# gitouni/Spatial-Temporal-LiDAR-camera-Calibration

Measured on NVIDIA B200. Metric: extrinsic_cost_evals_per_s, higher is better.
Workload: dtype f64

## Files before the change

### spatial-temporal-lidar-camera-calibration_b200/csrc/knn.cuh

```cuda
#pragma once
#include <cfloat>
#include <cmath>

#include "common.cuh"
#include "geom.cuh"
#include "kernels.h"

namespace stl {

constexpr unsigned kFull = 0xffffffffu;

struct ScanView {
    const float *px, *py, *pz;
    const uint32_t *orig;
    const float4 *lo, *hi;
    const uint16_t *adj;
    const float *adj_cov;
    unsigned long long *stats;
    int n0, n1;
};

__device__ __forceinline__ ScanView make_view(const DevPack &pk, const DevKf &K) {
    ScanView v;
    v.px = pk.px + K.pt_off; v.py = pk.py + K.pt_off; v.pz = pk.pz + K.pt_off;
    v.orig = pk.orig + K.pt_off;
    v.lo = pk.node_lo + K.node_off; v.hi = pk.node_hi + K.node_off;
    v.adj = pk.adj ? pk.adj + K.node_off * 32 : nullptr;
    v.adj_cov = pk.adj ? pk.adj_cov + K.node_off : nullptr;
    v.stats = nullptr;
    v.n0 = K.n0; v.n1 = K.n1;
    return v;
}

struct QueryF { float xl, xh, yl, yh, zl, zh; };
__device__ __forceinline__ QueryF make_queryf(double x, double y, double z) {
    QueryF q;
    q.xl = __double2float_rd(x); q.xh = __double2float_ru(x);
    q.yl = __double2float_rd(y); q.yh = __double2float_ru(y);
    q.zl = __double2float_rd(z); q.zh = __double2float_ru(z);
    return q;
}
__device__ __forceinline__ float box_lbf(const QueryF &q, float4 lo, float4 hi) {
    const float dx = fmaxf(fmaxf(__fsub_rd(lo.x, q.xh), __fsub_rd(q.xl, hi.x)), 0.f);
    const float dy = fmaxf(fmaxf(__fsub_rd(lo.y, q.yh), __fsub_rd(q.yl, hi.y)), 0.f);
    const float dz = fmaxf(fmaxf(__fsub_rd(lo.z, q.zh), __fsub_rd(q.zl, hi.z)), 0.f);
    const float s = __fadd_rd(__fadd_rd(__fmul_rd(dx, dx), __fmul_rd(dy, dy)), __fmul_rd(dz, dz));
    return __fmul_rd(s, 0.99999976f);
}

struct Sink1 {
    double d = DBL_MAX;
    float df = 3.402823466e+38f;
    float g2 = HUGE_VALF;
    uint32_t oi = 0xffffffffu, pos = 0xffffffffu;
    __device__ __forceinline__ bool may_contain(float lb) const { return lb <= df; }
    __device__ __forceinline__ static float below(double dd) { return __fmul_rd(__double2float_rd(dd), 0.99999976f); }
    __device__ __forceinline__ void note_pruned(float lb, bool pruned) {
        const unsigned k = __reduce_min_sync(kFull, pruned ? __float_as_uint(lb) : 0x7f800000u);
        g2 = fminf(g2, __uint_as_float(k));
    }
    __device__ __forceinline__ void note_bound(float b) { g2 = fminf(g2, b); }
    __device__ __forceinline__ void seed(const ScanView &S, uint32_t p, double qx, double qy, double qz) {
        const double dd = dist3e(qx, qy, qz, (double)S.px[p], (double)S.py[p], (double)S.pz[p]);
        if (dd == dd) { d = dd; df = __double2float_ru(dd); oi = S.orig[p]; pos = p; }
    }
    __device__ __forceinline__ void visit(const ScanView &S, int leaf, double qx, double qy, double qz, int lane) {
        const int g = leaf * kLeaf + lane;
        const double dd = dist3e(qx, qy, qz, (double)S.px[g], (double)S.py[g], (double)S.pz[g]);
        const float lowf = dd == dd ? below(dd) : __int_as_float(0x7f800000);
        const bool q = dd <= d;
        if (!__any_sync(kFull, q)) {
            note_pruned(lowf, (uint32_t)g != pos);
            return;
        }
        const uint32_t o = q ? S.orig[g] : 0xffffffffu;
        unsigned hi = q ? (unsigned)__double2hiint(dd) : 0xffffffffu;
        const unsigned mhi = __reduce_min_sync(kFull, hi);
        unsigned lo = (q && hi == mhi) ? (unsigned)__double2loint(dd) : 0xffffffffu;
        const unsigned mlo = __reduce_min_sync(kFull, lo);
        const bool tie = q && hi == mhi && (unsigned)__double2loint(dd) == mlo;
        const unsigned mo = __reduce_min_sync(kFull, tie ? o : 0xffffffffu);
        const double cd = __hiloint2double((int)mhi, (int)mlo);
        if (cd < d || (cd == d && mo < oi)) {
            const int src = __ffs(__ballot_sync(kFull, tie && o == mo)) - 1;
            if (pos != 0xffffffffu) g2 = fminf(g2, below(d));
            note_pruned(lowf, lane != src);
            d = cd; oi = mo; pos = (uint32_t)(leaf * kLeaf + src);
            df = __double2float_ru(cd);
        } else {
            note_pruned(lowf, (uint32_t)g != pos);
        }
    }
};

struct SinkK {
    double kd = DBL_MAX;
    uint32_t ki = 0xffffffffu, kpos = 0xffffffffu;
    int count = 0, k;
    double r2, wd;
    float r2f, wdf;
    uint32_t wi = 0xffffffffu;
    __device__ __forceinline__ SinkK(int k_, double r2_) : k(k_), r2(r2_), wd(r2_) {
        r2f = r2_ < 3.0e38 ? __double2float_ru(r2_) : 3.402823466e+38f;
        wdf = r2f;
    }
    __device__ __forceinline__ bool accept(double d, uint32_t i) const {
        return d < r2 && (count < k || d < wd || (d == wd && i < wi));
    }
    __device__ __forceinline__ bool may_contain(float lb) const { return lb <= r2f && (count < k || lb <= wdf); }
    __device__ __forceinline__ void note_pruned(float, bool) {}
    __device__ __forceinline__ void note_bound(float) {}
    __device__ __forceinline__ void visit(const ScanView &S, int leaf, double qx, double qy, double qz, int lane) {
        const int g = leaf * kLeaf + lane;
        const double dd = dist3e(qx, qy, qz, (double)S.px[g], (double)S.py[g], (double)S.pz[g]);
        const bool pre = dd < r2 && (count < k || dd <= wd);
        unsigned mask = __ballot_sync(kFull, pre);
        if (!mask) return;
        const uint32_t o = pre ? S.orig[g] : 0xffffffffu;
        if (__popc(mask) >= (count == 0 ? 4 : 8)) {
            bulk_merge(pre ? dd : (double)INFINITY, o, (uint32_t)g, lane);
            return;
        }
        while (mask) {
            const int src = __ffs(mask) - 1;
            mask &= mask - 1;
            const double cd = __shfl_sync(kFull, dd, src);
            const uint32_t ci = __shfl_sync(kFull, o, src);
            if (!accept(cd, ci)) continue;
            const bool less = lane < count && (kd < cd || (kd == cd && ki < ci));
            const int at = __popc(__ballot_sync(kFull, less));
            const double sd = __shfl_up_sync(kFull, kd, 1);
            const uint32_t si = __shfl_up_sync(kFull, ki, 1), sp = __shfl_up_sync(kFull, kpos, 1);
            if (lane > at) { kd = sd; ki = si; kpos = sp; }
            else if (lane == at) { kd = cd; ki = ci; kpos = (uint32_t)(leaf * kLeaf + src); }
            if (count < k) ++count;
            if (count == k) { wd = __shfl_sync(kFull, kd, k - 1); wi = __shfl_sync(kFull, ki, k - 1); wdf = __double2float_ru(wd); }
        }
    }

    __device__ __forceinline__ static void cx(double &d, uint32_t &i, uint32_t &p, int j, bool keep_min) {
        const double od = __shfl_xor_sync(kFull, d, j);
        const uint32_t oi = __shfl_xor_sync(kFull, i, j), op = __shfl_xor_sync(kFull, p, j);
        const bool other_less = od < d || (od == d && oi < i);
        const bool other_more = od > d || (od == d && oi > i);
        if (keep_min ? other_less : other_more) { d = od; i = oi; p = op; }
    }

    __device__ __forceinline__ void bulk_merge(double cd, uint32_t ci, uint32_t cp, int lane) {
        unsigned key = cd < (double)INFINITY ? ((__float_as_uint(__double2float_rd(cd)) & ~31u) | (unsigned)lane) : (0xffffffe0u | (unsigned)lane);
#pragma unroll
        for (int kk = 2; kk <= 32; kk <<= 1) {
#pragma unroll
            for (int j = kk >> 1; j > 0; j >>= 1) {
                const unsigned o = __shfl_xor_sync(kFull, key, j);
                const bool keep_min = ((lane & kk) == 0) == ((lane & j) == 0);
                key = keep_min ? min(key, o) : max(key, o);
            }
        }
        {
            const int src = (int)(key & 31u);
            const double sd = __shfl_sync(kFull, cd, src);
            const uint32_t si = __shfl_sync(kFull, ci, src), sp = __shfl_sync(kFull, cp, src);
            cd = sd; ci = si; cp = sp;
        }
        const unsigned next_key = __shfl_down_sync(kFull, key, 1);
        if (__ballot_sync(kFull, lane < 31 && (key >> 5) == (next_key >> 5) && cd < (double)INFINITY)) {
            for (;;) {
                bool moved = false;
#pragma unroll 1
                for (int parity = 0; parity < 2; ++parity) {
                    const bool lower = (lane & 1) == parity;
                    const int partner = lower ? lane + 1 : lane - 1;
                    const bool ok = partner >= 0 && partner < 32;
                    const double od = __shfl_sync(kFull, cd, ok ? partner : lane);
                    const uint32_t oi = __shfl_sync(kFull, ci, ok ? partner : lane), op = __shfl_sync(kFull, cp, ok ? partner : lane);
                    const bool other_less = od < cd || (od == cd && oi < ci);
                    const bool other_more = od > cd || (od == cd && oi > ci);
                    if (ok && (lower ? other_less : other_more)) { cd = od; ci = oi; cp = op; moved = true; }
                }
                if (!__any_sync(kFull, moved)) break;
            }
        }
        if (count == 0) {
            kd = cd; ki = ci; kpos = cp;
        } else {
            if (lane >= count) { kd = (double)INFINITY; ki = 0xffffffffu; }
            const double rd = __shfl_sync(kFull, cd, 31 - lane);
            const uint32_t ri = __shfl_sync(kFull, ci, 31 - lane), rp = __shfl_sync(kFull, cp, 31 - lane);
            if (rd < kd || (rd == kd && ri < ki)) { kd = rd; ki = ri; kpos = rp; }
#pragma unroll
            for (int j = 16; j > 0; j >>= 1) cx(kd, ki, kpos, j, (lane & j) == 0);
        }
        const int nvalid = __popc(__ballot_sync(kFull, kd < (double)INFINITY));
        count = nvalid < k ? nvalid : k;
        if (count == k) { wd = __shfl_sync(kFull, kd, k - 1); wi = __shfl_sync(kFull, ki, k - 1); wdf = __double2float_ru(wd); }
    }
};

template <class Sink>
__device__ __forceinline__ void traverse(const ScanView &S, double qx, double qy, double qz, Sink &sink, int lane, int first_leaf = -1) {
    if (first_leaf >= 0) sink.visit(S, first_leaf, qx, qy, qz, lane);
    const float4 *lo2 = S.lo + S.n0 + S.n1, *hi2 = S.hi + S.n0 + S.n1;
    const float4 *lo1 = S.lo + S.n0, *hi1 = S.hi + S.n0;
    const QueryF qf = make_queryf(qx, qy, qz);
    const float lb2 = box_lbf(qf, lo2[lane], hi2[lane]);
    const unsigned key2 = __float_as_uint(lb2);
    unsigned done2 = 0;
    for (;;) {
        const bool c2 = !((done2 >> lane) & 1u) && sink.may_contain(lb2);
        const unsigned m2 = __reduce_min_sync(kFull, c2 ? key2 : 0xffffffffu);
        if (m2 == 0xffffffffu) break;
        const int s2 = __ffs(__ballot_sync(kFull, c2 && key2 == m2)) - 1;
        done2 |= 1u << s2;
        const int n1i = s2 * 32 + lane;
        const float lb1 = box_lbf(qf, lo1[n1i], hi1[n1i]);
        const unsigned key1 = __float_as_uint(lb1);
        unsigned done1 = 0;
        for (;;) {
                const bool c1 = !((done1 >> lane) & 1u) && sink.may_contain(lb1);
            const unsigned m1 = __reduce_min_sync(kFull, c1 ? key1 : 0xffffffffu);
            if (m1 == 0xffffffffu) break;
            const int s1 = __ffs(__ballot_sync(kFull, c1 && key1 == m1)) - 1;
            done1 |= 1u << s1;
            const int n0i = (s2 * 32 + s1) * 32 + lane;
            const float lb0 = box_lbf(qf, S.lo[n0i], S.hi[n0i]);
            const unsigned key0 = __float_as_uint(lb0);
            unsigned done0 = ((s2 * 32 + s1) == (first_leaf >> 5) && first_leaf >= 0) ? (1u << (first_leaf & 31)) : 0u;
            for (;;) {
                        const bool c0 = !((done0 >> lane) & 1u) && sink.may_contain(lb0);
                const unsigned m0 = __reduce_min_sync(kFull, c0 ? key0 : 0xffffffffu);
                if (m0 == 0xffffffffu) break;
                const int s0 = __ffs(__ballot_sync(kFull, c0 && key0 == m0)) - 1;
                done0 |= 1u << s0;
                sink.visit(S, (s2 * 32 + s1) * 32 + s0, qx, qy, qz, lane);
            }
            sink.note_pruned(lb0, !((done0 >> lane) & 1u));
        }
        sink.note_pruned(lb1, !((done1 >> lane) & 1u));
    }
    sink.note_pruned(lb2, !((done2 >> lane) & 1u));
}

__device__ __forceinline__ int next_ticket(int *ticket, int lane) {
    int t = 0;
    if (lane == 0) t = atomicAdd(ticket, 1);
    return __shfl_sync(kFull, t, 0);
}

template <class Sink>
__device__ __forceinline__ float scan_adjacent(const ScanView &S, int home, double qx, double qy, double qz, Sink &sink, int lane) {
    if (S.adj == nullptr) return -1.f;
    const float cov = S.adj_cov[home];
    if (cov < 0.f) return -1.f;
    const unsigned id = S.adj[(long long)home * 32 + lane];
    const QueryF qf = make_queryf(qx, qy, qz);
    const float lb = id != 0xffffu ? box_lbf(qf, S.lo[id], S.hi[id]) : __int_as_float(0x7f800000);
    const unsigned key = __float_as_uint(lb);
    unsigned done = 0;
    for (;;) {
        const bool c = !((done >> lane) & 1u) && sink.may_contain(lb);
        const unsigned m = __reduce_min_sync(kFull, c ? key : 0xffffffffu);
        if (m == 0xffffffffu) break;
        const int s = __ffs(__ballot_sync(kFull, c && key == m)) - 1;
        done |= 1u << s;
        sink.visit(S, (int)__shfl_sync(kFull, id, s), qx, qy, qz, lane);
    }
    sink.note_pruned(lb, !((done >> lane) & 1u));
    return cov;
}

__device__ __forceinline__ void knn_around_point(const ScanView &S, uint32_t pos, SinkK &kn, int lane) {
    const double x = (double)S.px[pos], y = (double)S.py[pos], z = (double)S.pz[pos];
    const float cov = scan_adjacent(S, (int)(pos >> 5), x, y, z, kn, lane);
    const bool done = cov > 3.0e38f || (cov >= 0.f && kn.count == kn.k && kn.wdf < cov);
    if (S.stats && lane == 0) { atomicAdd(S.stats + 0, 1ull); atomicAdd(S.stats + (done ? 1 : (cov >= 0.f ? 2 : 3)), 1ull); }
    if (done) return;
    if (cov >= 0.f) kn = SinkK(kn.k, kn.r2);
    traverse(S, x, y, z, kn, lane, (int)(pos >> 5));
}

__device__ __forceinline__ float home_box_delta(const ScanView &S, int home, double qx, double qy, double qz) {
    const float4 lo = S.lo[home], hi = S.hi[home];
    const float xl = __double2float_rd(qx), xh = __double2float_ru(qx), yl = __double2float_rd(qy), yh = __double2float_ru(qy);
    const float zl = __double2float_rd(qz), zh = __double2float_ru(qz);
    const float gx = fmaxf(fmaxf(__fsub_ru(lo.x, xl), __fsub_ru(xh, hi.x)), 0.f);
    const float gy = fmaxf(fmaxf(__fsub_ru(lo.y, yl), __fsub_ru(yh, hi.y)), 0.f);
    const float gz = fmaxf(fmaxf(__fsub_ru(lo.z, zl), __fsub_ru(zh, hi.z)), 0.f);
    return __fsqrt_ru(__fadd_ru(__fadd_ru(__fmul_ru(gx, gx), __fmul_ru(gy, gy)), __fmul_ru(gz, gz)));
}

__device__ __forceinline__ void nn_near_leaf_seeded(const ScanView &S, float adj_r, int home, double qx, double qy, double qz, Sink1 &nn,
                                                    int lane, float delta) {
    const float cov = scan_adjacent(S, home, qx, qy, qz, nn, lane);
    if (S.stats && lane == 0) atomicAdd(S.stats + 4, 1ull);
    if (cov >= 0.f && nn.pos != 0xffffffffu) {
        const float reach = __fadd_ru(__fsqrt_ru(nn.df), delta);
        if (cov > 3.0e38f ? reach <= adj_r : reach < __fsqrt_rd(cov)) {
            if (S.stats && lane == 0) atomicAdd(S.stats + 5, 1ull);
            const float u = __fsub_rd(cov > 3.0e38f ? adj_r : __fsqrt_rd(cov), delta);
            nn.note_bound(u > 0.f ? __fmul_rd(u, u) : 0.f);
            return;
        }
        const int l1 = (int)(nn.pos >> 5);
        if (l1 != home) {
            const float cov1 = S.adj_cov[l1];
            const float two_rho = __fmul_ru(2.f, __fsqrt_ru(nn.df));
            if (cov1 >= 0.f && (cov1 > 3.0e38f ? two_rho <= adj_r : two_rho < __fsqrt_rd(cov1))) {
                const float rho_up = __fsqrt_ru(nn.df);
                scan_adjacent(S, l1, qx, qy, qz, nn, lane);
                if (S.stats && lane == 0) atomicAdd(S.stats + 5, 1ull);
                const float u = __fsub_rd(cov1 > 3.0e38f ? adj_r : __fsqrt_rd(cov1), rho_up);
                nn.note_bound(u > 0.f ? __fmul_rd(u, u) : 0.f);
                return;
            }
        }
    }
    if (S.stats && lane == 0) atomicAdd(S.stats + (cov >= 0.f ? 6 : 7), 1ull);
    traverse(S, qx, qy, qz, nn, lane);
}

__device__ __forceinline__ void nn_near_leaf(const ScanView &S, float adj_r, int home, double qx, double qy, double qz, Sink1 &nn,
                                             int lane, uint32_t hint = 0xffffffffu) {
    if (hint != 0xffffffffu) nn.seed(S, hint, qx, qy, qz);
    nn_near_leaf_seeded(S, adj_r, home, qx, qy, qz, nn, lane, home_box_delta(S, home, qx, qy, qz));
}

struct PlaneOut { V3 n; double reg; int m; bool gates_ok; };

struct NbGather {
    const ScanView &S;
    const uint32_t *__restrict__ nb;
    __device__ __forceinline__ void get(int j, double &x, double &y, double &z) const {
        const uint32_t p = nb[j];
        x = (double)S.px[p]; y = (double)S.py[p]; z = (double)S.pz[p];
    }
};
struct NbCoords {
    const float4 *__restrict__ base;
    long long stride;
    __device__ __forceinline__ void get(int j, double &x, double &y, double &z) const {
        const float4 v = base[(long long)j * stride];
        x = (double)v.x; y = (double)v.y; z = (double)v.z;
    }
};
__device__ __forceinline__ void store_nb_coords(float4 *__restrict__ nbx, long long stride, long long slot, const ScanView &S, int lane,
                                                int count, uint32_t kpos) {
    float4 v = make_float4(0.f, 0.f, 0.f, 0.f);
    if (lane < count) v = make_float4(S.px[kpos], S.py[kpos], S.pz[kpos], __uint_as_float(kpos));
    nbx[(long long)lane * stride + slot] = v;
}

template <class Src>
__device__ __forceinline__ PlaneOut plane_fit(const Src &src, int m, double last, double cx, double cy, double cz, const DevParams &pr,
                                              const bool stable = false) {
    PlaneOut out;
    out.m = m;
    out.n = {0.0, 0.0, 0.0};
    out.reg = 0;
    out.gates_ok = false;
    if (stable) {
        if (m < 3) return out;
    } else if (m == 0 || (last < pr.min_diff2) || (m < pr.min_pts)) {
        return out;
    }
    out.gates_ok = true;
    double c0 = 0, c1 = 0, c2 = 0, c3 = 0, c4 = 0, c5 = 0, c6 = 0, c7 = 0, c8 = 0;
    for (int j = 0; j < m; ++j) {
        double x, y, z;
        src.get(j, x, y, z);
        c0 += x; c1 += y; c2 += z;
        c3 += x * x; c4 += x * y; c5 += x * z;
        c6 += y * y; c7 += y * z; c8 += z * z;
    }
    const double dm = (double)m;
    c0 /= dm; c1 /= dm; c2 /= dm; c3 /= dm; c4 /= dm; c5 /= dm; c6 /= dm; c7 /= dm; c8 /= dm;
    const double cov[6] = {c3 - c0 * c0, c4 - c0 * c1, c5 - c0 * c2, c6 - c1 * c1, c7 - c1 * c2, c8 - c2 * c2};
    const V3 n = normalized(smallest_eigvec(cov));
    double reg = 0;
    for (int j = 0; j < m; ++j) {
        double x, y, z;
        src.get(j, x, y, z);
        const V3 d = {x - cx, y - cy, z - cz};
        reg += fabs(dot(d, n));
    }
    out.n = n;
    out.reg = reg / (double)(m - 1);
    if (stable && sqrt(last) < pr.min_diff) out.reg = __longlong_as_double(0x7ff0000000000000ll);
    return out;
}


__device__ __forceinline__ PlaneOut plane_thread(const ScanView &S, const uint32_t *__restrict__ nb, int m, double last, double cx,
                                                 double cy, double cz, const DevParams &pr, const bool stable = false) {
    return plane_fit(NbGather{S, nb}, m, last, cx, cy, cz, pr, stable);
}

__device__ __forceinline__ PlaneOut plane_lookup(const DevPack &pk, const DevKf &K, uint32_t pos) {
    const PlaneRec r = pk.pl_rec[K.pt_off + pos];
    const int mm = pk.pl_m[K.pt_off + pos];
    PlaneOut out;
    out.gates_ok = mm >= 0;
    out.m = mm >= 0 ? mm : -(mm + 1);
    out.n = {r.nx, r.ny, r.nz};
    out.reg = r.reg;
    return out;
}

}
```

### spatial-temporal-lidar-camera-calibration_b200/csrc/knn3d.cu

```cuda
#include <algorithm>
#include <cstdlib>

#include "kernels.h"
#include "knn.cuh"

namespace stl {
namespace {

constexpr int kWarps = 8;
#ifndef STL_KNN_MINB
#define STL_KNN_MINB 8
#endif
constexpr int kPlaneThreads = 128;
#ifndef STL_PLANE_MINB
#define STL_PLANE_MINB 5
#endif

__device__ __forceinline__ void map_point_lidar(const DevPack &pk, const DevKf &K, const DevCand &c, int f, uint32_t kp, double &qx,
                                                double &qy, double &qz) {
    const float *Tcw = pk.Tcw + (long long)f * 12;
    const float *mp = pk.kp_mp + (K.kp_off + kp) * 3;
    const double wx = (double)__fmul_rn(mp[0], c.sf), wy = (double)__fmul_rn(mp[1], c.sf), wz = (double)__fmul_rn(mp[2], c.sf);
    const double cxm = dadd(dot3e((double)Tcw[0], (double)Tcw[1], (double)Tcw[2], wx, wy, wz), dmul((double)Tcw[3], c.s));
    const double cym = dadd(dot3e((double)Tcw[4], (double)Tcw[5], (double)Tcw[6], wx, wy, wz), dmul((double)Tcw[7], c.s));
    const double czm = dadd(dot3e((double)Tcw[8], (double)Tcw[9], (double)Tcw[10], wx, wy, wz), dmul((double)Tcw[11], c.s));
    xform(c.Ri, c.ti, cxm, cym, czm, qx, qy, qz);
}

__global__ void __launch_bounds__(kWarps * 32, STL_KNN_MINB)
k_nn_knn(const DevPack pk, const DevWork wk, const DevParams pr, const int B, const int batch, uint32_t *__restrict__ lm_pos,
         int *__restrict__ lm_m) {
    const int sub = wk.sub;
    const int j = blockIdx.x % sub;
    const int bf = blockIdx.x / sub;
    const int fi = bf / B, f = sel_kf(pk, fi), b = bf - fi * B;
    const int nq = wk.n_q[(long long)b * pk.n_kf + f];
    if (nq <= 0) return;
    const int lane = threadIdx.x & 31;
    const DevKf K = pk.kf[f];
    const DevCand &c = wk.cand[b];
    ScanView S = make_view(pk, K);
    S.stats = wk.dbg_stats;
    const long long cbase = (long long)b * pk.n_kp_total + K.kp_off;
    const long long qbase = (long long)b * pk.n_mp_total + K.mp_off;
    __shared__ int ticket;
    if (threadIdx.x == 0) ticket = 0;
    __syncthreads();
    for (;;) {
        const int t0 = next_ticket(&ticket, lane) * batch;
        if ((long long)t0 * sub + j >= nq) break;
        const int qi = (t0 + lane) * sub + j;
        const bool valid = lane < batch && qi < nq;
        double qx = 0, qy = 0, qz = 0, sd = DBL_MAX;
        uint32_t hint = 0, soi = 0xffffffffu, spos = 0xffffffffu;
        float delta = 0.f;
        if (valid) {
            const uint2 ks = wk.q_kpsp[cbase + qi];
            hint = ks.y;
            map_point_lidar(pk, K, c, f, ks.x, qx, qy, qz);
            const double dd = dist3e(qx, qy, qz, (double)S.px[hint], (double)S.py[hint], (double)S.pz[hint]);
            if (dd == dd) { sd = dd; soi = S.orig[hint]; spos = hint; }
            delta = home_box_delta(S, (int)(hint >> 5), qx, qy, qz);
        }
        uint32_t out_pos = 0xffffffffu;
        float out_g2 = 0.f;
        unsigned todo = __ballot_sync(kFull, valid);
        while (todo) {
            const int src = __ffs(todo) - 1;
            todo &= todo - 1;
            const double x = __shfl_sync(kFull, qx, src), y = __shfl_sync(kFull, qy, src), z = __shfl_sync(kFull, qz, src);
            const uint32_t h = __shfl_sync(kFull, hint, src);
            Sink1 nn;
            nn.d = __shfl_sync(kFull, sd, src);
            nn.oi = __shfl_sync(kFull, soi, src);
            nn.pos = __shfl_sync(kFull, spos, src);
            if (nn.pos != 0xffffffffu) nn.df = __double2float_ru(nn.d);
            nn_near_leaf_seeded(S, pr.adj_r, (int)(h >> 5), x, y, z, nn, lane, __shfl_sync(kFull, delta, src));
            if (lane == src) { out_pos = nn.pos; out_g2 = nn.g2; }
            if (pr.use_plane && !pr.plane_index) {
                const long long slot = qbase + (long long)(t0 + src) * sub + j;
                SinkK kn(pr.k, pr.radius2);
                knn_around_point(S, nn.pos, kn, lane);
                wk.nb[slot * kMaxK + lane] = lane < kn.count ? kn.kpos : 0xffffffffu;
                store_nb_coords(wk.nbx, wk.nbx_stride, slot, S, lane, kn.count, kn.kpos);
                const double last = __shfl_sync(kFull, kn.kd, kn.count > 0 ? kn.count - 1 : 0);
                if (lane == 0) { wk.nb_m[slot] = kn.count; wk.nb_last[slot] = last; }
            }
        }
        if (valid) { wk.nn_pos[qbase + qi] = out_pos; wk.nn_g2[qbase + qi] = out_g2; }
        if (lm_pos != nullptr && b == 0) {
            double lx = 0, ly = 0, lz = 0, nn_d = DBL_MAX;
            uint32_t nn_p = 0xffffffffu;
            bool need = false;
            if (valid) {
                const float *Tcw = pk.Tcw + (long long)f * 12;
                const float *mp = pk.kp_mp + (K.kp_off + wk.q_kpsp[cbase + qi].x) * 3;
                const double ma = (double)mp[0], mb = (double)mp[1], mc = (double)mp[2];
                const double Mx = dadd(dot3e((double)Tcw[0], (double)Tcw[1], (double)Tcw[2], ma, mb, mc), (double)Tcw[3]);
                const double My = dadd(dot3e((double)Tcw[4], (double)Tcw[5], (double)Tcw[6], ma, mb, mc), (double)Tcw[7]);
                const double Mz = dadd(dot3e((double)Tcw[8], (double)Tcw[9], (double)Tcw[10], ma, mb, mc), (double)Tcw[11]);
                xform(c.Ri, c.ti, dmul(Mx, c.s), dmul(My, c.s), dmul(Mz, c.s), lx, ly, lz);
                need = true;
                if (out_pos != 0xffffffffu) {
                    const double move = sqrt(dist3e(qx, qy, qz, lx, ly, lz)) * (1.0 + 1e-9) + 1e-12;
                    const double dh = dist3e(lx, ly, lz, (double)S.px[out_pos], (double)S.py[out_pos], (double)S.pz[out_pos]);
                    const double reach = (double)__fsqrt_rd(out_g2) - move;
                    if (reach > 0.0 && reach * reach > dh * (1.0 + 1e-6) + 1e-18) { need = false; nn_p = out_pos; nn_d = dh; }
                }
            }
            unsigned todo2 = __ballot_sync(kFull, need);
            while (todo2) {
                const int src = __ffs(todo2) - 1;
                todo2 &= todo2 - 1;
                const double x = __shfl_sync(kFull, lx, src), y = __shfl_sync(kFull, ly, src), z = __shfl_sync(kFull, lz, src);
                uint32_t h = __shfl_sync(kFull, out_pos, src);
                if (h == 0xffffffffu) h = __shfl_sync(kFull, hint, src);
                Sink1 nn;
                nn_near_leaf(S, pr.adj_r, (int)(h >> 5), x, y, z, nn, lane, h);
                if (lane == src) { nn_p = nn.pos; nn_d = nn.d; }
            }
            if (valid) {
                const long long slot = K.mp_off + qi;
                if (nn_d > pr.max_3d_dist2) {
                    lm_pos[slot] = 0xffffffffu;
                } else {
                    lm_pos[slot] = nn_p;
                    lm_m[slot] = nn_p == hint ? -2 : -3;
                }
            }
        }
    }
}

__global__ void __launch_bounds__(kPlaneThreads, STL_PLANE_MINB)
k_plane_dist(const DevPack pk, const DevWork wk, const DevParams pr, const int B, const int debug) {
    const int sub = wk.sub;
    const int j = blockIdx.x % sub;
    const int bf = blockIdx.x / sub;
    const int fi = bf / B, f = sel_kf(pk, fi), b = bf - fi * B;
    const long long rec = (long long)b * pk.n_kf + f;
    const int nq = wk.n_q[rec];
    double s3d = 0, v3d = 0, c3d = 0, vpl = 0, vpt = 0;
    if (nq > 0) {
        const DevKf K = pk.kf[f];
        const DevCand &c = wk.cand[b];
        const ScanView S = make_view(pk, K);
        const long long cbase = (long long)b * pk.n_kp_total + K.kp_off;
        const long long qbase = (long long)b * pk.n_mp_total + K.mp_off;
        for (int qi = j * kPlaneThreads + threadIdx.x; qi < nq; qi += sub * kPlaneThreads) {
            const uint32_t kp = wk.corr_kp[cbase + wk.q_corr[cbase + qi]];
            double qx, qy, qz;
            map_point_lidar(pk, K, c, f, kp, qx, qy, qz);
            const uint32_t np = wk.nn_pos[qbase + qi];
            const double nx = (double)S.px[np], ny = (double)S.py[np], nz = (double)S.pz[np];
            const double dx = dsub(nx, qx), dy = dsub(ny, qy), dz = dsub(nz, qz);
            double dist = sqrt(dot3e(dx, dy, dz, dx, dy, dz));
            int is_plane = 0, m = 0;
            if (pr.use_plane) {
                const PlaneOut po = pr.plane_index ? plane_lookup(pk, K, np)
                                                   : plane_fit(NbCoords{wk.nbx + qbase + qi, wk.nbx_stride}, wk.nb_m[qbase + qi], wk.nb_last[qbase + qi], nx, ny, nz, pr, pr.variant == 1);
                m = po.m;
                if (po.gates_ok && !(po.reg > pr.reg_thr)) {
                    is_plane = 1;
                    dist = fabs(dot3e(dx, dy, dz, po.n.x, po.n.y, po.n.z));
                }
            }
            if (dist < pr.thr3d) {
                s3d += dist; v3d += 1.0;
                if (is_plane) vpl += 1.0; else vpt += 1.0;
            }
            c3d += 1.0;
            if (debug) {
                const long long o = K.kp_off + qi;
                wk.dbg_nn[o] = S.orig[np];
                wk.dbg_m[o] = m;
                wk.dbg_plane[o] = is_plane;
                wk.dbg_dist[o] = dist;
                for (int t = 0; t < kMaxK; ++t) {
                    const uint32_t p = (pr.use_plane && !pr.plane_index && t < m) ? wk.nb[(qbase + qi) * kMaxK + t] : 0xffffffffu;
                    wk.dbg_knn[o * kMaxK + t] = p == 0xffffffffu ? 0xffffffffu : S.orig[p];
                }
            }
        }
    }
    __shared__ double red[5][kPlaneThreads / 32];
    const int lane = threadIdx.x & 31, warp = threadIdx.x >> 5;
    for (int o = 16; o; o >>= 1) {
        s3d += __shfl_down_sync(0xffffffffu, s3d, o); v3d += __shfl_down_sync(0xffffffffu, v3d, o);
        c3d += __shfl_down_sync(0xffffffffu, c3d, o); vpl += __shfl_down_sync(0xffffffffu, vpl, o);
        vpt += __shfl_down_sync(0xffffffffu, vpt, o);
    }
    if (lane == 0) { red[0][warp] = s3d; red[1][warp] = v3d; red[2][warp] = c3d; red[3][warp] = vpl; red[4][warp] = vpt; }
    __syncthreads();
    if (threadIdx.x == 0) {
        AlignRec r = {0, 0, 0, 0, 0};
        for (int w = 0; w < kPlaneThreads / 32; ++w) { r.s3d += red[0][w]; r.v3d += red[1][w]; r.c3d += red[2][w]; r.vpl += red[3][w]; r.vpt += red[4][w]; }
        wk.align[rec * sub + j] = r;
    }
}

__global__ void __launch_bounds__(kWarps * 32)
k_knn3d(const DevPack pk, const int kf, const double *__restrict__ q, const int nq, const int k, const double radius2,
        uint32_t *__restrict__ out_idx, double *__restrict__ out_d2, int *__restrict__ out_cnt) {
    const int lane = threadIdx.x & 31;
    const int qi = blockIdx.x * kWarps + (threadIdx.x >> 5);
    if (qi >= nq) return;
    const DevKf K = pk.kf[kf];
    const ScanView S = make_view(pk, K);
    SinkK kn(k, radius2 > 0 ? radius2 : DBL_MAX);
    traverse(S, q[qi * 3], q[qi * 3 + 1], q[qi * 3 + 2], kn, lane);
    if (lane < k) {
        out_idx[(long long)qi * k + lane] = lane < kn.count ? kn.ki : 0xffffffffu;
        out_d2[(long long)qi * k + lane] = lane < kn.count ? kn.kd : INFINITY;
    }
    if (lane == 0) out_cnt[qi] = kn.count;
}

__global__ void __launch_bounds__(kWarps * 32, STL_KNN_MINB)
k_index_knn(const DevPack pk, const int kf_begin, const DevParams pr, const long long first_pt, uint32_t *__restrict__ nb,
            int *__restrict__ nb_m, double *__restrict__ nb_last) {
    const DevKf K = pk.kf[kf_begin + blockIdx.y];
    const int lane = threadIdx.x & 31, warp = threadIdx.x >> 5;
    const ScanView S = make_view(pk, K);
    for (int p = blockIdx.x * kWarps + warp; p < K.n_pts; p += gridDim.x * kWarps) {
        SinkK kn(pr.k, pr.radius2);
        knn_around_point(S, (uint32_t)p, kn, lane);
        const long long o = K.pt_off - first_pt + p;
        nb[o * kMaxK + lane] = lane < kn.count ? kn.kpos : 0xffffffffu;
        const double last = __shfl_sync(kFull, kn.kd, kn.count > 0 ? kn.count - 1 : 0);
        if (lane == 0) { nb_m[o] = kn.count; nb_last[o] = last; }
    }
}

__global__ void __launch_bounds__(kPlaneThreads)
k_index_plane(const DevPack pk, const int kf_begin, const DevParams pr, const long long first_pt, const uint32_t *__restrict__ nb,
              const int *__restrict__ nb_m, const double *__restrict__ nb_last) {
    const DevKf K = pk.kf[kf_begin + blockIdx.y];
    const ScanView S = make_view(pk, K);
    for (int p = blockIdx.x * kPlaneThreads + threadIdx.x; p < K.n_pad; p += gridDim.x * kPlaneThreads) {
        PlaneRec r = {0.0, 0.0, 0.0, 0.0};
        int mm = -1;
        if (p < K.n_pts) {
            const long long o = K.pt_off - first_pt + p;
            const PlaneOut po = plane_thread(S, nb + o * kMaxK, nb_m[o], nb_last[o], (double)S.px[p], (double)S.py[p], (double)S.pz[p], pr, pr.variant == 1);
            r.nx = po.n.x; r.ny = po.n.y; r.nz = po.n.z; r.reg = po.reg;
            mm = po.gates_ok ? po.m : -(po.m + 1);
        }
        pk.pl_rec[K.pt_off + p] = r;
        pk.pl_m[K.pt_off + p] = mm;
    }
}

}

cudaError_t build_plane_index(const DevPack &pk, const DevKf *h_kf, int kf_begin, int nkf, const DevParams &pr, cudaStream_t st,
                              BuildScratch &scr) {
    const long long first = h_kf[kf_begin].pt_off;
    const long long npts = h_kf[kf_begin + nkf - 1].pt_off + h_kf[kf_begin + nkf - 1].n_pad - first;
    if (npts <= 0) return cudaSuccess;
    int max_pts = 0;
    for (int f = 0; f < nkf; ++f) max_pts = max_pts > h_kf[kf_begin + f].n_pad ? max_pts : h_kf[kf_begin + f].n_pad;
    cudaError_t e = scr.need(2, 4 * (size_t)npts * kMaxK);
    if (e == cudaSuccess) e = scr.need(4, 4 * (size_t)npts);
    if (e == cudaSuccess) e = scr.need(3, 8 * (size_t)npts);
    if (e != cudaSuccess) return e;
    uint32_t *nb = (uint32_t *)scr.buf[2]; int *m = (int *)scr.buf[4]; double *last = (double *)scr.buf[3];
    const int bx = (max_pts + kWarps * 16 - 1) / (kWarps * 16);
    k_index_knn<<<dim3(bx, nkf), kWarps * 32, 0, st>>>(pk, kf_begin, pr, first, nb, m, last);
    k_index_plane<<<dim3((max_pts + kPlaneThreads * 4 - 1) / (kPlaneThreads * 4), nkf), kPlaneThreads, 0, st>>>(pk, kf_begin, pr, first, nb, m, last);
    return cudaGetLastError();
}

namespace {
__global__ void k_debug_trig(const double *__restrict__ x, int n, double *__restrict__ ac, double *__restrict__ co) {
    const int i = blockIdx.x * blockDim.x + threadIdx.x;
    if (i >= n) return;
    ac[i] = acos_cr(fmin(fmax(x[i], -1.0), 1.0));
    co[i] = cos_cr(x[i]);
}
}

cudaError_t launch_debug_trig(const double *d_x, int n, double *d_acos, double *d_cos, cudaStream_t st) {
    if (n <= 0) return cudaSuccess;
    k_debug_trig<<<(n + 255) / 256, 256, 0, st>>>(d_x, n, d_acos, d_cos);
    return cudaGetLastError();
}

cudaError_t launch_align3d(const DevPack &pk, const DevWork &wk, const DevParams &pr, int B, int debug, cudaStream_t st, cudaEvent_t after_traversal,
                           uint32_t *lm_pos, int *lm_m) {
    if (B <= 0) return cudaSuccess;
    if (pk.n_sel <= 0) return after_traversal ? cudaEventRecord(after_traversal, st) : cudaSuccess;
    int batch = (long long)pk.n_sel * B >= 600 ? 8 : 4;
    if (const char *e = getenv("STL_K2_BATCH")) batch = std::max(1, std::min(32, atoi(e)));
    k_nn_knn<<<(unsigned)(pk.n_sel * B * wk.sub), kWarps * 32, 0, st>>>(pk, wk, pr, B, batch, lm_pos, lm_m);
    cudaError_t e = cudaGetLastError();
    if (e != cudaSuccess) return e;
    if (after_traversal && (e = cudaEventRecord(after_traversal, st)) != cudaSuccess) return e;
    k_plane_dist<<<(unsigned)(pk.n_sel * B * wk.sub), kPlaneThreads, 0, st>>>(pk, wk, pr, B, debug);
    return cudaGetLastError();
}

cudaError_t launch_knn3d(const DevPack &pk, int kf, const double *d_q, int nq, int k, double radius2, uint32_t *d_idx, double *d_d2,
                         int *d_cnt, cudaStream_t st) {
    if (nq <= 0) return cudaSuccess;
    k_knn3d<<<(nq + kWarps - 1) / kWarps, kWarps * 32, 0, st>>>(pk, kf, d_q, nq, k, radius2, d_idx, d_d2, d_cnt);
    return cudaGetLastError();
}

}
```

### spatial-temporal-lidar-camera-calibration_b200/csrc/lm.cu

```cuda
#include <cub/cub.cuh>

#include "../../include/stlcalib.h"
#include "dual.cuh"
#include "gprfit.hpp"
#include "knn.cuh"
#include "lm.h"

namespace stl {
namespace {

constexpr int kWarps = 8;
#ifndef STL_LM_MINB
#define STL_LM_MINB 6
#endif
constexpr int kLinVals = 41;
constexpr int kGprWarps = 1;
constexpr int kLinThreads = 128;


__device__ __forceinline__ void lm_lane(const DevPack &pk, DevWork &wk, LmState &lm, bool arg0 = true) {
    const int2 am = arg0 && blockIdx.y == 0 ? lm.lane0 : lm.amap[blockIdx.y];
    const long long nk = pk.n_kp_total, F = pk.n_kf, nm = lm.n_slots;
    const long long wc = am.x, wq = wc * nm;
    wk.cand += wc;
    wk.corr_kp += wc * nk; wk.corr_sp += wc * nk; wk.q_corr += wc * nk; wk.q_kpsp += wc * nk;
    wk.n_corr += wc * F; wk.n_q += wc * F;
    wk.nn_pos += wq; wk.nn_g2 += wq; wk.nb += wq * kMaxK; wk.nbx += wq; wk.nb_m += wq; wk.nb_last += wq;
    const long long lo = (long long)blockIdx.y * nm;
    lm.stage += lo; lm.plane_a += lo * 4; lm.nnb_pos += lo; lm.nbb += lo * kMaxK; lm.nbbx += lo; lm.nbb_m += lo; lm.nbb_last += lo;
    const long long po = (long long)am.y * lm.slot_stride;
    lm.slot_kf += po; lm.slot_kp += po; lm.flag2d += po; lm.type3d += po; lm.flag3d += po; lm.flagG += po;
    lm.geo2d += po * 6; lm.geo3d += po * 9; lm.gpr_nb += po * kMaxK; lm.gpr_m += po;
    lm.d_counts += am.y * 4;
}

__global__ void k_lm_clear(LmState lm) {
    const long long po = (long long)lm.amap[blockIdx.y].y * lm.slot_stride, n = lm.slot_stride, ptot = (long long)lm.P * n;
    for (long long i = (long long)blockIdx.x * blockDim.x + threadIdx.x; i < n; i += (long long)gridDim.x * blockDim.x) {
        lm.flags[po + i] = 0; lm.flags[ptot + po + i] = 0; lm.flags[2 * ptot + po + i] = 0; lm.flags[3 * ptot + po + i] = 0;
    }
    if (blockIdx.x == 0 && threadIdx.x < 4) lm.d_counts[lm.amap[blockIdx.y].y * 4 + threadIdx.x] = 0;
}

__device__ __forceinline__ bool lm_frame_active(const DevWork &wk, const DevParams &pr, int f, int &nq) {
    nq = wk.n_q[f];
    return wk.n_corr[f] >= pr.num_min_corr && nq > 0;
}

__device__ __forceinline__ void lm_map_point(const DevPack &pk, const DevKf &K, int f, uint32_t kp, double &Mx, double &My, double &Mz) {
    const float *Tcw = pk.Tcw + (long long)f * 12;
    const float *mp = pk.kp_mp + (K.kp_off + kp) * 3;
    const double a = (double)mp[0], b = (double)mp[1], c = (double)mp[2];
    Mx = dadd(dot3e((double)Tcw[0], (double)Tcw[1], (double)Tcw[2], a, b, c), (double)Tcw[3]);
    My = dadd(dot3e((double)Tcw[4], (double)Tcw[5], (double)Tcw[6], a, b, c), (double)Tcw[7]);
    Mz = dadd(dot3e((double)Tcw[8], (double)Tcw[9], (double)Tcw[10], a, b, c), (double)Tcw[11]);
}

__global__ void __launch_bounds__(kWarps * 32, STL_LM_MINB)
k_lm_knn_a(const DevPack pk, DevWork wk, const DevParams pr, LmState lm) {
    lm_lane(pk, wk, lm);
    const int j = blockIdx.x % lm.sub, f = sel_kf(pk, blockIdx.x / lm.sub);
    int nq;
    if (!lm_frame_active(wk, pr, f, nq)) return;
    const int lane = threadIdx.x & 31, warp = threadIdx.x >> 5;
    const DevKf K = pk.kf[f];
    const ScanView S = make_view(pk, K);
    const int C = pk.n_covis;
    __shared__ int ticket;
    if (threadIdx.x == 0) ticket = 0;
    __syncthreads();
    for (;;) {
        const int qi = next_ticket(&ticket, lane) * lm.sub + j;
        if (qi >= nq) break;
        const uint2 ks = wk.q_kpsp[K.kp_off + qi];
        const uint32_t kp = ks.x, sp = ks.y;
        const long long slot = K.mp_off + qi;
        const bool obs = lane < C && pk.covis_valid[f * C + lane] && !isnan(pk.covis_uv[(K.kp_off + kp) * C + lane].x);
        const int ncov = __popc(__ballot_sync(kFull, obs));
        if (ncov == 0) {
            if (lane == 0) wk.nb_m[slot] = -1;
            continue;
        }
        if (pr.plane_index && !pr.use_gpr) {
            if (lane == 0) wk.nb_m[slot] = 0;
            continue;
        }
        SinkK kn(pr.k, pr.radius2);
        knn_around_point(S, sp, kn, lane);
        wk.nb[slot * kMaxK + lane] = lane < kn.count ? kn.kpos : 0xffffffffu;
        store_nb_coords(wk.nbx, wk.nbx_stride, slot, S, lane, kn.count, kn.kpos);
        const double last = __shfl_sync(kFull, kn.kd, kn.count > 0 ? kn.count - 1 : 0);
        if (lane == 0) { wk.nb_m[slot] = kn.count; wk.nb_last[slot] = last; }
    }
}

__global__ void __launch_bounds__(128)
k_lm_plane_a(const DevPack pk, DevWork wk, const DevParams pr, LmState lm) {
    lm_lane(pk, wk, lm);
    const int j = blockIdx.x % lm.sub, f = sel_kf(pk, blockIdx.x / lm.sub);
    int nq;
    if (!lm_frame_active(wk, pr, f, nq)) return;
    __shared__ int cnt[2];
    if (threadIdx.x < 2) cnt[threadIdx.x] = 0;
    __syncthreads();
    const DevKf K = pk.kf[f];
    const ScanView S = make_view(pk, K);
    const bool from_index = pr.plane_index && !pr.use_gpr;
    const int C = pk.n_covis;
    for (int qi = j * blockDim.x + threadIdx.x; qi < nq; qi += lm.sub * blockDim.x) {
        const long long slot = K.mp_off + qi;
        lm.stage[slot] = 0;
        const uint32_t ci = wk.q_corr[K.kp_off + qi];
        const uint32_t kp = wk.corr_kp[K.kp_off + ci], sp = wk.corr_sp[K.kp_off + ci];
        int m = 0;
        if (from_index) {
            bool any = false;
            for (int s = 0; s < C; ++s) any = any || (pk.covis_valid[f * C + s] && !isnan(pk.covis_uv[(K.kp_off + kp) * C + s].x));
            if (!any) continue;
        } else {
            m = wk.nb_m[slot];
            if (m < 0) continue;
        }
        const double cx = (double)S.px[sp], cy = (double)S.py[sp], cz = (double)S.pz[sp];
        const PlaneOut po = from_index ? plane_lookup(pk, K, sp)
                                       : plane_fit(NbCoords{wk.nbx + slot, wk.nbx_stride}, m, wk.nb_last[slot], cx, cy, cz, pr);
        if (!po.gates_ok) continue;
        const long long cs = slot;
        lm.slot_kf[cs] = f;
        lm.slot_kp[cs] = kp;
        double *pa = lm.plane_a + slot * 4;
        pa[0] = po.n.x; pa[1] = po.n.y; pa[2] = po.n.z; pa[3] = po.reg;
        if (po.reg < pr.reg_thr) {
            double *g = lm.geo2d + cs * 6;
            g[0] = cx; g[1] = cy; g[2] = cz; g[3] = po.n.x; g[4] = po.n.y; g[5] = po.n.z;
            lm.flag2d[cs] = 1;
            atomicAdd(&cnt[0], 1);
        } else if (pr.use_gpr) {
            for (int t = 0; t < kMaxK; ++t) lm.gpr_nb[slot * kMaxK + t] = wk.nb[slot * kMaxK + t];
            lm.gpr_m[slot] = po.m;
            lm.flagG[cs] = 1;
            atomicAdd(&cnt[1], 1);
        }
        lm.stage[slot] = 1;
    }
    __syncthreads();
    if (threadIdx.x < 2 && cnt[threadIdx.x] > 0) atomicAdd(lm.d_counts + 3 * threadIdx.x, cnt[threadIdx.x]);
}

__global__ void __launch_bounds__(kWarps * 32, STL_LM_MINB)
k_lm_knn_b(const DevPack pk, DevWork wk, const DevParams pr, LmState lm, const bool hints, const bool cert) {
    lm_lane(pk, wk, lm);
    const uint32_t *__restrict__ nn_hint = hints ? wk.nn_pos : nullptr;
    const float *__restrict__ nn_g2 = hints && cert ? wk.nn_g2 : nullptr;
    const int j = blockIdx.x % lm.sub, f = sel_kf(pk, blockIdx.x / lm.sub);
    int nq;
    if (!lm_frame_active(wk, pr, f, nq)) return;
    const int lane = threadIdx.x & 31;
    const DevKf K = pk.kf[f];
    const DevCand &c0 = wk.cand[0];
    const ScanView S = make_view(pk, K);
    const float *Tcw = pk.Tcw + (long long)f * 12;
    __shared__ int ticket;
    if (threadIdx.x == 0) ticket = 0;
    __syncthreads();
    for (;;) {
        const int base = next_ticket(&ticket, lane) * 32;
        if ((long long)base * lm.sub + j >= nq) break;
        const int qi = (base + lane) * lm.sub + j;
        const long long slot = K.mp_off + qi;
        const bool valid = qi < nq && lm.stage[slot] == 1;
        uint32_t sp = 0, hint = 0xffffffffu, nn_pos = 0xffffffffu;
        double qx = 0, qy = 0, qz = 0, nn_d = DBL_MAX;
        bool settled = false;
        if (valid) {
            const uint2 ks = wk.q_kpsp[K.kp_off + qi];
            const uint32_t kp = ks.x;
            sp = ks.y;
            double Mx, My, Mz;
            lm_map_point(pk, K, f, kp, Mx, My, Mz);
            xform(c0.Ri, c0.ti, dmul(Mx, c0.s), dmul(My, c0.s), dmul(Mz, c0.s), qx, qy, qz);
            hint = nn_hint ? nn_hint[slot] : sp;
            if (hint == 0xffffffffu) hint = sp;
            if (nn_hint && nn_g2 && nn_hint[slot] != 0xffffffffu) {
                const float *mp = pk.kp_mp + (K.kp_off + kp) * 3;
                const double wx = (double)__fmul_rn(mp[0], c0.sf), wy = (double)__fmul_rn(mp[1], c0.sf), wz = (double)__fmul_rn(mp[2], c0.sf);
                const double ex = dadd(dot3e((double)Tcw[0], (double)Tcw[1], (double)Tcw[2], wx, wy, wz), dmul((double)Tcw[3], c0.s));
                const double ey = dadd(dot3e((double)Tcw[4], (double)Tcw[5], (double)Tcw[6], wx, wy, wz), dmul((double)Tcw[7], c0.s));
                const double ez = dadd(dot3e((double)Tcw[8], (double)Tcw[9], (double)Tcw[10], wx, wy, wz), dmul((double)Tcw[11], c0.s));
                double ox, oy, oz;
                xform(c0.Ri, c0.ti, ex, ey, ez, ox, oy, oz);
                const double move = sqrt(dist3e(ox, oy, oz, qx, qy, qz)) * (1.0 + 1e-9) + 1e-12;
                const double dh = dist3e(qx, qy, qz, (double)S.px[hint], (double)S.py[hint], (double)S.pz[hint]);
                const double reach = (double)__fsqrt_rd(nn_g2[slot]) - move;
                if (reach > 0.0 && reach * reach > dh * (1.0 + 1e-6) + 1e-18) { settled = true; nn_pos = hint; nn_d = dh; }
            }
        }
        unsigned todo = __ballot_sync(kFull, valid && !settled);
        while (todo) {
            const int src = __ffs(todo) - 1;
            todo &= todo - 1;
            const double sx = __shfl_sync(kFull, qx, src), sy = __shfl_sync(kFull, qy, src), sz = __shfl_sync(kFull, qz, src);
            const uint32_t sh = __shfl_sync(kFull, hint, src);
            Sink1 nn;
            nn_near_leaf(S, pr.adj_r, (int)(sh >> 5), sx, sy, sz, nn, lane, sh);
            if (lane == src) { nn_pos = nn.pos; nn_d = nn.d; }
        }
        bool want_knn = false;
        if (valid) {
            if (nn_d > pr.max_3d_dist2) {
                lm.nnb_pos[slot] = 0xffffffffu;
            } else {
                lm.nnb_pos[slot] = nn_pos;
                if (nn_pos == sp) lm.nbb_m[slot] = -2;
                else if (pr.plane_index) lm.nbb_m[slot] = -3;
                else want_knn = true;
            }
        }
        unsigned kn_todo = __ballot_sync(kFull, want_knn);
        while (kn_todo) {
            const int src = __ffs(kn_todo) - 1;
            kn_todo &= kn_todo - 1;
            const uint32_t p = __shfl_sync(kFull, nn_pos, src);
            const long long sl = K.mp_off + ((long long)(base + src) * lm.sub + j);
            SinkK kn(pr.k, pr.radius2);
            knn_around_point(S, p, kn, lane);
            lm.nbb[sl * kMaxK + lane] = lane < kn.count ? kn.kpos : 0xffffffffu;
            store_nb_coords(lm.nbbx, lm.nbbx_stride, sl, S, lane, kn.count, kn.kpos);
            const double last = __shfl_sync(kFull, kn.kd, kn.count > 0 ? kn.count - 1 : 0);
            if (lane == 0) { lm.nbb_m[sl] = kn.count; lm.nbb_last[sl] = last; }
        }
    }
}

__device__ __forceinline__ bool block3d_geometry(const DevPack &pk, const DevParams &pr, const LmState &lm, long long slot, int f, uint32_t kp,
                                                 double g[9], int &type) {
    if (lm.stage[slot] != 1) return false;
    const uint32_t np = lm.nnb_pos[slot];
    if (np == 0xffffffffu) return false;
    const DevKf &K = pk.kf[f];
    const float *sx = pk.px + K.pt_off, *sy = pk.py + K.pt_off, *sz = pk.pz + K.pt_off;
    const double nx = (double)sx[np], ny = (double)sy[np], nz = (double)sz[np];
    bool gates_ok, state;
    double n3[3];
    const int m = lm.nbb_m[slot];
    if (m == -2) {
        const double *pa = lm.plane_a + slot * 4;
        gates_ok = true; n3[0] = pa[0]; n3[1] = pa[1]; n3[2] = pa[2];
        state = pa[3] < pr.reg_thr;
    } else {
        const PlaneOut p2 = m == -3 ? plane_lookup(pk, K, np) : plane_fit(NbCoords{lm.nbbx + slot, lm.nbbx_stride}, m, lm.nbb_last[slot], nx, ny, nz, pr);
        gates_ok = p2.gates_ok; n3[0] = p2.n.x; n3[1] = p2.n.y; n3[2] = p2.n.z;
        state = p2.gates_ok && p2.reg < pr.reg_thr;
    }
    lm_map_point(pk, K, f, kp, g[0], g[1], g[2]);
    g[3] = nx; g[4] = ny; g[5] = nz;
    g[6] = gates_ok ? n3[0] : 0.0; g[7] = gates_ok ? n3[1] : 0.0; g[8] = gates_ok ? n3[2] : 1.0;
    type = state ? 2 : 1;
    return true;
}

__global__ void __launch_bounds__(128)
k_lm_plane_b(const DevPack pk, DevWork wk, const DevParams pr, LmState lm) {
    lm_lane(pk, wk, lm, false);
    const int j = blockIdx.x % lm.sub, f = sel_kf(pk, blockIdx.x / lm.sub);
    int nq;
    if (!lm_frame_active(wk, pr, f, nq)) return;
    const DevKf K = pk.kf[f];
    __shared__ int cnt[2];
    if (threadIdx.x < 2) cnt[threadIdx.x] = 0;
    __syncthreads();
    for (int qi = j * blockDim.x + threadIdx.x; qi < nq; qi += lm.sub * blockDim.x) {
        const long long slot = K.mp_off + qi;
        if (lm.stage[slot] != 1) continue;
        if (lm.nnb_pos[slot] == 0xffffffffu) continue;
        const uint32_t ci = wk.q_corr[K.kp_off + qi];
        const uint32_t kp = wk.corr_kp[K.kp_off + ci];
        double g9[9];
        int type;
        if (!block3d_geometry(pk, pr, lm, slot, f, kp, g9, type)) continue;
        double *g = lm.geo3d + slot * 9;
#pragma unroll
        for (int i = 0; i < 9; ++i) g[i] = g9[i];
        lm.type3d[slot] = (uint8_t)type;
        lm.flag3d[slot] = 1;
        atomicAdd(&cnt[0], 1);
        if (type == 1) atomicAdd(&cnt[1], 1);
    }
    __syncthreads();
    if (threadIdx.x < 2 && cnt[threadIdx.x] > 0) atomicAdd(lm.d_counts + 1 + threadIdx.x, cnt[threadIdx.x]);
}

struct Acc {
    double v[kLinVals];
};

struct F7 {
    double a;
    double v[7];
};
static_assert(sizeof(F7) == sizeof(D7), "F7 views D7 storage");
__device__ __forceinline__ F7 f7_const(double x) { F7 r; r.a = x; for (int i = 0; i < 7; ++i) r.v[i] = 0.0; return r; }
__device__ __forceinline__ F7 operator+(const F7 &f, const F7 &g) { F7 r; r.a = f.a + g.a; for (int i = 0; i < 7; ++i) r.v[i] = f.v[i] + g.v[i]; return r; }
__device__ __forceinline__ F7 operator-(const F7 &f, const F7 &g) { F7 r; r.a = f.a - g.a; for (int i = 0; i < 7; ++i) r.v[i] = f.v[i] - g.v[i]; return r; }
__device__ __forceinline__ F7 operator*(const F7 &f, const F7 &g) { F7 r; r.a = f.a * g.a; for (int i = 0; i < 7; ++i) r.v[i] = fma(f.a, g.v[i], f.v[i] * g.a); return r; }
__device__ __forceinline__ F7 operator/(const F7 &f, const F7 &g) {
    F7 r;
    const double gi = 1.0 / g.a, q = f.a * gi;
    r.a = q;
    for (int i = 0; i < 7; ++i) r.v[i] = fma(-q, g.v[i], f.v[i]) * gi;
    return r;
}
__device__ __forceinline__ F7 operator*(const F7 &f, double c) { F7 r; r.a = f.a * c; for (int i = 0; i < 7; ++i) r.v[i] = f.v[i] * c; return r; }
__device__ __forceinline__ F7 operator+(const F7 &f, double c) { F7 r = f; r.a = f.a + c; return r; }
__device__ __forceinline__ F7 operator-(const F7 &f, double c) { F7 r = f; r.a = f.a - c; return r; }

__device__ __forceinline__ void huber(double sq, double delta, double &rho0, double &sr) {
    if (sq > delta * delta) {
        const double r = sqrt(sq);
        rho0 = 2.0 * delta * r - delta * delta;
        sr = sqrt(fmax(DBL_MIN, delta / r));
    } else {
        rho0 = sq;
        sr = 1.0;
    }
}

__device__ __forceinline__ void accumulate(Acc &A, const D7 &e, double sr) {
    const double r = sr * e.a;
    double J[7];
#pragma unroll
    for (int a = 0; a < 7; ++a) J[a] = sr * e.v[a];
    int h = 8;
#pragma unroll
    for (int a = 0; a < 7; ++a) {
        A.v[1 + a] += J[a] * r;
#pragma unroll
        for (int b = a; b < 7; ++b) A.v[h++] += J[a] * J[b];
    }
}

__device__ __forceinline__ void mv3(const D7 *M, const D7 *p, D7 *o) {
#pragma unroll
    for (int i = 0; i < 3; ++i) o[i] = (M[i * 3] * p[0] + M[i * 3 + 1] * p[1]) + M[i * 3 + 2] * p[2];
}
__device__ __forceinline__ void mv3(const F7 *M, const F7 *p, F7 *o) {
#pragma unroll
    for (int i = 0; i < 3; ++i) o[i] = (M[i * 3] * p[0] + M[i * 3 + 1] * p[1]) + M[i * 3 + 2] * p[2];
}
__device__ __forceinline__ void accumulate(Acc &A, const F7 &e, double sr) {
    const double r = sr * e.a;
    double J[7];
#pragma unroll
    for (int a = 0; a < 7; ++a) J[a] = sr * e.v[a];
    int h = 8;
#pragma unroll
    for (int a = 0; a < 7; ++a) {
        A.v[1 + a] = fma(J[a], r, A.v[1 + a]);
#pragma unroll
        for (int b = a; b < 7; ++b) { A.v[h] = fma(J[a], J[b], A.v[h]); ++h; }
    }
}

template <class T7>
__device__ __forceinline__ void put_row(const BlockOut &o, long long blk, int r, const T7 &e) {
    o.res[blk * o.rmax + r] = e.a;
    double *j = o.jac + (blk * o.rmax + r) * 7;
#pragma unroll
    for (int a = 0; a < 7; ++a) j[a] = e.v[a];
}
__device__ __forceinline__ void put_head(const BlockOut &o, long long blk, int type, int kf, uint32_t kp, int nres) {
    o.type[blk] = type; o.kf[blk] = kf; o.kp[blk] = (int32_t)kp; o.nres[blk] = nres;
}

__device__ __forceinline__ void lm_list_start(const LmState &lm, int p, int which, int *out) {
    if (threadIdx.x >= 32) return;
    int s = 0;
    for (int q = threadIdx.x; q < p; q += 32) s += lm.d_counts[q * 4 + which];
    for (int o = 16; o; o >>= 1) s += __shfl_down_sync(0xffffffffu, s, o);
    if (threadIdx.x == 0) *out = s;
}

__device__ __forceinline__ int sel_slot(const DevPack &pk, int v) {
    int lo = 0, hi = pk.n_sel;
    while (hi - lo > 1) {
        const int mid = (lo + hi) >> 1;
        if (pk.sel_mp[mid].x <= v) lo = mid; else hi = mid;
    }
    return v + pk.sel_mp[lo].y;
}

template <bool WB>
__global__ void __launch_bounds__(kLinThreads)
k_linearize(const DevPack pk, const DevParams pr, const LmState lm, const LmCand *__restrict__ cands, const int *__restrict__ cprob,
            double *__restrict__ partial, int partial_stride, const BlockOut bo) {
    __shared__ LmCand c;
    __shared__ int list0;
    const int prob = cprob ? cprob[blockIdx.y] : 0;
    {
        const double *src = reinterpret_cast<const double *>(cands + blockIdx.y);
        double *dst = reinterpret_cast<double *>(&c);
        for (int i = threadIdx.x; i < (int)(sizeof(LmCand) / 8); i += kLinThreads) dst[i] = src[i];
    }
    lm_list_start(lm, prob, 0, &list0);
    __syncthreads();
    const F7 *cR = reinterpret_cast<const F7 *>(c.R), *ct = reinterpret_cast<const F7 *>(c.t);
    const F7 *cRlc = reinterpret_cast<const F7 *>(c.Rlc), *ctlc = reinterpret_cast<const F7 *>(c.tlc);
    const F7 &cs7 = *reinterpret_cast<const F7 *>(&c.s);
    Acc A;
#pragma unroll
    for (int i = 0; i < kLinVals; ++i) A.v[i] = 0.0;
    const int C = pk.n_covis;
    const int stride = gridDim.x * kLinThreads, t0 = blockIdx.x * kLinThreads + threadIdx.x;

    const int *counts = lm.d_counts + prob * 4;
    const int n2d = counts[0];
    const int *idx2d = lm.idx2d + list0;
    for (int it = t0; it < n2d; it += stride) {
        const int slot = idx2d[it];
        const int f = lm.slot_kf[slot];
        const uint32_t kp = lm.slot_kp[slot];
        const DevKf &K = pk.kf[f];
        const double fx = K.fx, fy = K.fy, cx = K.cx, cy = K.cy;
        const float2 kxy = pk.kp_xy[K.kp_off + kp];
        const double *g = lm.geo2d + (long long)slot * 6;
        const F7 p0[3] = {f7_const(g[0]), f7_const(g[1]), f7_const(g[2])}, n0[3] = {f7_const(g[3]), f7_const(g[4]), f7_const(g[5])};
        F7 p0c[3], n0c[3];
        mv3(cR, p0, p0c);
#pragma unroll
        for (int i = 0; i < 3; ++i) p0c[i] = p0c[i] + ct[i];
        mv3(cR, n0, n0c);
        const double Cxz = ((double)kxy.x - cx) / fx, Cyz = ((double)kxy.y - cy) / fy;
        const F7 num = (n0c[0] * p0c[0] + n0c[1] * p0c[1]) + n0c[2] * p0c[2];
        const F7 den = (n0c[0] * Cxz + n0c[1] * Cyz) + n0c[2];
        const F7 Z0 = num / den;
        const F7 P0[3] = {Z0 * Cxz, Z0 * Cyz, Z0};
        double sq = 0.0;
        int nres = 0;
        for (int s = 0; s < C; ++s) {
            if (!pk.covis_valid[f * C + s]) continue;
            const float2 uv = pk.covis_uv[(K.kp_off + kp) * C + s];
            if (isnan(uv.x)) continue;
            const float *rp = pk.relpose + ((long long)f * C + s) * 12;
            double P1[3];
#pragma unroll
            for (int i = 0; i < 3; ++i)
                P1[i] = (((double)rp[i * 4] * P0[0].a + (double)rp[i * 4 + 1] * P0[1].a) + (double)rp[i * 4 + 2] * P0[2].a) + (double)rp[i * 4 + 3] * c.s.a;
            const double eu = (fx * P1[0] / P1[2] + cx) - (double)uv.x, ev = (fy * P1[1] / P1[2] + cy) - (double)uv.y;
            sq += eu * eu;
            sq += ev * ev;
            nres += 2;
        }
        double rho0, sr;
        huber(sq, pr.delta2d, rho0, sr);
        A.v[0] += 0.5 * rho0;
        A.v[36] += 1.0;
        A.v[39] += (double)nres;
        int wrow = 0;
        for (int s = 0; s < C; ++s) {
            if (!pk.covis_valid[f * C + s]) continue;
            const float2 uv = pk.covis_uv[(K.kp_off + kp) * C + s];
            if (isnan(uv.x)) continue;
            const float *rp = pk.relpose + ((long long)f * C + s) * 12;
            F7 P1[3];
#pragma unroll
            for (int i = 0; i < 3; ++i)
                P1[i] = ((P0[0] * (double)rp[i * 4] + P0[1] * (double)rp[i * 4 + 1]) + P0[2] * (double)rp[i * 4 + 2]) + cs7 * (double)rp[i * 4 + 3];
            const F7 eu = ((P1[0] * fx) / P1[2] + cx) - (double)uv.x;
            const F7 ev = ((P1[1] * fy) / P1[2] + cy) - (double)uv.y;
            accumulate(A, eu, sr);
            accumulate(A, ev, sr);
            if (WB) { put_row(bo, it, wrow, eu); put_row(bo, it, wrow + 1, ev); wrow += 2; }
        }
        if (WB) put_head(bo, it, 0, f, kp, nres);
    }

    const long long n3 = WB ? (long long)counts[1] : (pk.sel ? pk.n_sel_mp : lm.max_blocks);
    const long long po = (long long)prob * lm.slot_stride;
    const uint8_t *flag3d = lm.flag3d + po, *type3d = lm.type3d + po;
    const double *geo3d = lm.geo3d + po * 9;
    __shared__ int q3[kLinThreads / 32][64];
    const int lane3 = threadIdx.x & 31, warp3 = threadIdx.x >> 5;
    int qlen = 0;
    long long base = (long long)blockIdx.x * kLinThreads + warp3 * 32;
    for (long long it = t0;; it += stride) {
        long long slot = it;
        if (WB) {
            if (it >= n3) break;
            slot = lm.idx3d[it];
        } else {
            const bool more = base < n3;
            if (more) {
                const long long sl = base + lane3;
                const int rs = pk.sel && sl < n3 ? sel_slot(pk, (int)sl) : (int)sl;
                const bool on = sl < n3 && flag3d[rs];
                const unsigned mask = __ballot_sync(0xffffffffu, on);
                if (on) q3[warp3][qlen + __popc(mask & ((1u << lane3) - 1))] = rs;
                qlen += __popc(mask);
                base += stride;
                __syncwarp();
            }
            if (qlen < 32 && more) continue;
            if (qlen == 0) break;
            const int take = qlen < 32 ? qlen : 32;
            const int mine = lane3 < take ? q3[warp3][lane3] : -1;
            const int rest = lane3 + 32 < qlen ? q3[warp3][lane3 + 32] : 0;
            __syncwarp();
            if (lane3 + 32 < qlen) q3[warp3][lane3] = rest;
            qlen -= take;
            __syncwarp();
            if (mine < 0) continue;
            slot = mine;
        }
        const double *g = geo3d + slot * 9;
        const int type = type3d[slot];
        const F7 Ms[3] = {cs7 * g[0], cs7 * g[1], cs7 * g[2]};
        F7 M[3];
        mv3(cRlc, Ms, M);
#pragma unroll
        for (int i = 0; i < 3; ++i) M[i] = M[i] + ctlc[i];
        const F7 d[3] = {M[0] - g[3], M[1] - g[4], M[2] - g[5]};
        double rho0, sr;
        if (type == 1) {
            huber((d[0].a * d[0].a + d[1].a * d[1].a) + d[2].a * d[2].a, pr.delta3d, rho0, sr);
            accumulate(A, d[0], sr);
            accumulate(A, d[1], sr);
            accumulate(A, d[2], sr);
            A.v[37] += 1.0;
            A.v[39] += 3.0;
            if (WB) {
                const long long blk = (long long)n2d + it;
                put_row(bo, blk, 0, d[0]); put_row(bo, blk, 1, d[1]); put_row(bo, blk, 2, d[2]);
                put_head(bo, blk, 1, lm.slot_kf[po + slot], lm.slot_kp[po + slot], 3);
            }
        } else {
            const F7 e = (d[0] * g[6] + d[1] * g[7]) + d[2] * g[8];
            huber(e.a * e.a, pr.delta3d, rho0, sr);
            accumulate(A, e, sr);
            A.v[38] += 1.0;
            A.v[39] += 1.0;
            if (WB) {
                const long long blk = (long long)n2d + it;
                put_row(bo, blk, 0, e);
                put_head(bo, blk, 2, lm.slot_kf[po + slot], lm.slot_kp[po + slot], 1);
            }
        }
        A.v[0] += 0.5 * rho0;
    }

    __shared__ double red[kLinThreads / 32][kLinVals];
    const int lane = threadIdx.x & 31, warp = threadIdx.x >> 5;
#pragma unroll
    for (int i = 0; i < kLinVals; ++i) {
        double x = A.v[i];
        for (int o = 16; o; o >>= 1) x += __shfl_down_sync(0xffffffffu, x, o);
        if (lane == 0) red[warp][i] = x;
    }
    __syncthreads();
    if (threadIdx.x < kLinVals) {
        double x = 0.0;
        for (int w = 0; w < kLinThreads / 32; ++w) x += red[w][threadIdx.x];
        partial[((long long)blockIdx.y * partial_stride + blockIdx.x) * kLinVals + threadIdx.x] = x;
    }
}


constexpr int kGprTri = 32 * 33 / 2;
struct GprSmem {
    double L[8][kGprTri];
    double xu[8][32], xv[8][32], y[8][32];
    double al[8][32];
};

__device__ __forceinline__ int tri(int i, int j) { return i * (i + 1) / 2 + j; }
__device__ __forceinline__ D7 ld7(const double (*m)[kGprTri], int idx) {
    D7 r; r.a = m[0][idx];
#pragma unroll
    for (int c = 0; c < 7; ++c) r.v[c] = m[1 + c][idx];
    return r;
}
__device__ __forceinline__ void st7(double (*m)[kGprTri], int idx, const D7 &x) {
    m[0][idx] = x.a;
#pragma unroll
    for (int c = 0; c < 7; ++c) m[1 + c][idx] = x.v[c];
}
__device__ __forceinline__ D7 ld7v(const double (*m)[32], int i) {
    D7 r; r.a = m[0][i];
#pragma unroll
    for (int c = 0; c < 7; ++c) r.v[c] = m[1 + c][i];
    return r;
}
__device__ __forceinline__ void st7v(double (*m)[32], int i, const D7 &x) {
    m[0][i] = x.a;
#pragma unroll
    for (int c = 0; c < 7; ++c) m[1 + c][i] = x.v[c];
}
__device__ __forceinline__ D7 d7_sqrt_dev(const D7 &f) {
    D7 r; r.a = sqrt(f.a);
    const double t = 1.0 / (2.0 * r.a);
#pragma unroll
    for (int c = 0; c < 7; ++c) r.v[c] = t * f.v[c];
    return r;
}
__device__ __forceinline__ D7 d7_exp_dev(const D7 &f) {
    D7 r; r.a = exp(f.a);
#pragma unroll
    for (int c = 0; c < 7; ++c) r.v[c] = r.a * f.v[c];
    return r;
}
__device__ __forceinline__ D7 shfl7(const D7 &x, int src) {
    D7 r; r.a = __shfl_sync(0xffffffffu, x.a, src);
#pragma unroll
    for (int c = 0; c < 7; ++c) r.v[c] = __shfl_sync(0xffffffffu, x.v[c], src);
    return r;
}

template <bool WB>
__global__ void __launch_bounds__(32)
k_linearize_gpr(const DevPack pk, const DevParams pr, const LmState lm, const LmCand *__restrict__ cands, const int *__restrict__ cprob,
                double *__restrict__ partial, int partial_stride, int partial_off, const BlockOut bo) {
    __shared__ GprSmem S;
    __shared__ LmCand c;
    __shared__ int list0;
    const int lane = threadIdx.x;
    const int prob = cprob ? cprob[blockIdx.y] : 0;
    {
        const double *src = reinterpret_cast<const double *>(cands + blockIdx.y);
        double *dst = reinterpret_cast<double *>(&c);
        for (int i = lane; i < (int)(sizeof(LmCand) / 8); i += 32) dst[i] = src[i];
    }
    lm_list_start(lm, prob, 3, &list0);
    __syncwarp();
    const int *counts = lm.d_counts + prob * 4;
    Acc A;
#pragma unroll
    for (int i = 0; i < kLinVals; ++i) A.v[i] = 0.0;
    const int C = pk.n_covis;
    const int nG = counts[3];
    for (int it = blockIdx.x; it < nG; it += gridDim.x) {
        const int cs = lm.idxG[list0 + it];
        const int f = lm.slot_kf[cs];
        const uint32_t kp = lm.slot_kp[cs];
        const long long gblk = (long long)counts[0] + counts[1] + it;
        const long long ms = cs;
        const int n = lm.gpr_m[ms];
        const DevKf &K = pk.kf[f];
        const double fx = K.fx, fy = K.fy, cx = K.cx, cy = K.cy;
        const float2 kxy = pk.kp_xy[K.kp_off + kp];
        const double u0 = kxy.x, v0 = kxy.y;
        const double sigma = lm.gpr_hyper ? lm.gpr_hyper[ms * 2] : pr.gpr_sigma, ell = lm.gpr_hyper ? lm.gpr_hyper[ms * 2 + 1] : pr.gpr_l;
        const double sigma2 = sigma * sigma;
        const double inv_l2 = 1.0 / (ell * ell);
        const double coef = -0.5 * inv_l2;
        const D7 kdiag = d7_const(sigma2 * exp(coef * 0.0) + pr.gpr_noise);
        __syncwarp();
        D7 myu = d7_const(0.0), myv = d7_const(0.0);
        if (lane < n) {
            const uint32_t p = lm.gpr_nb[ms * kMaxK + lane];
            const double px = (double)pk.px[K.pt_off + p], py = (double)pk.py[K.pt_off + p], pz = (double)pk.pz[K.pt_off + p];
            D7 tf[3];
#pragma unroll
            for (int i = 0; i < 3; ++i) tf[i] = ((c.R[i * 3] * px + c.R[i * 3 + 1] * py) + c.R[i * 3 + 2] * pz) + c.t[i];
            myu = (tf[0] * fx) / tf[2] + cx;
            myv = (tf[1] * fy) / tf[2] + cy;
            st7v(S.xu, lane, myu); st7v(S.xv, lane, myv); st7v(S.y, lane, tf[2]);
        }
        __syncwarp();
        if (lane < n) {
            for (int j = 0; j < lane; ++j) {
                const D7 dx = ld7v(S.xu, j) - myu, dy = ld7v(S.xv, j) - myv;
                const D7 kv = d7_exp_dev((dx * dx + dy * dy) * coef) * sigma2;
                st7(S.L, tri(lane, j), kv);
            }
            st7(S.L, tri(lane, lane), kdiag);
        }
        __syncwarp();
        for (int k = 0; k < n; ++k) {
            D7 v = d7_const(0.0);
            if (lane >= k && lane < n) {
                v = ld7(S.L, tri(lane, k));
                for (int j = 0; j < k; ++j) v = v - ld7(S.L, tri(lane, j)) * ld7(S.L, tri(k, j));
            }
            D7 xk = shfl7(v, k);
            xk = d7_sqrt_dev(xk);
            if (lane == k) st7(S.L, tri(k, k), xk);
            else if (lane > k && lane < n) st7(S.L, tri(lane, k), v / xk);
            __syncwarp();
        }
        {
            D7 v = lane < n ? ld7v(S.y, lane) : d7_const(0.0);
            for (int j = 0; j < n; ++j) {
                D7 aj = v / ld7(S.L, tri(min(lane, n - 1), min(lane, n - 1)));
                aj = shfl7(aj, j);
                if (lane == j) v = aj;
                else if (lane > j && lane < n) v = v - ld7(S.L, tri(lane, j)) * aj;
            }
            if (lane < n) st7v(S.al, lane, v);
            __syncwarp();
            for (int i = n - 1; i >= 0; --i) {
                if (lane == i) {
                    D7 w = ld7v(S.al, i);
                    for (int j = i + 1; j < n; ++j) w = w - ld7(S.L, tri(j, i)) * ld7v(S.al, j);
                    st7v(S.al, i, w / ld7(S.L, tri(i, i)));
                }
                __syncwarp();
            }
        }
        D7 term = d7_const(0.0);
        if (lane < n) {
            const D7 dx = myu - u0, dy = myv - v0;
            const D7 ks = d7_exp_dev((dx * dx + dy * dy) * (-0.5 * inv_l2)) * sigma2;
            term = ks * ld7v(S.al, lane);
        }
        D7 z = d7_const(0.0);
        for (int j = 0; j < n; ++j) z = z + shfl7(term, j);
        if (lane == 0) {
            const double ifx = 1.0 / fx, ify = 1.0 / fy;
            const D7 P0[3] = {(z * (u0 - cx)) * ifx, (z * (v0 - cy)) * ify, z};
            double sq = 0.0;
            int nres = 0;
            for (int s = 0; s < C; ++s) {
                if (!pk.covis_valid[f * C + s]) continue;
                const float2 uv = pk.covis_uv[(K.kp_off + kp) * C + s];
                if (isnan(uv.x)) continue;
                const float *rp = pk.relpose + ((long long)f * C + s) * 12;
                double P1[3];
                for (int i = 0; i < 3; ++i)
                    P1[i] = (((double)rp[i * 4] * P0[0].a + (double)rp[i * 4 + 1] * P0[1].a) + (double)rp[i * 4 + 2] * P0[2].a) + (double)rp[i * 4 + 3] * c.s.a;
                const double eu = (fx * P1[0] / P1[2] + cx) - (double)uv.x, ev = (fy * P1[1] / P1[2] + cy) - (double)uv.y;
                sq += eu * eu;
                sq += ev * ev;
                nres += 2;
            }
            double rho0, sr;
            huber(sq, pr.delta2d, rho0, sr);
            A.v[0] += 0.5 * rho0;
            A.v[40] += 1.0;
            A.v[39] += (double)nres;
            int wrow = 0;
            for (int s = 0; s < C; ++s) {
                if (!pk.covis_valid[f * C + s]) continue;
                const float2 uv = pk.covis_uv[(K.kp_off + kp) * C + s];
                if (isnan(uv.x)) continue;
                const float *rp = pk.relpose + ((long long)f * C + s) * 12;
                D7 P1[3];
                for (int i = 0; i < 3; ++i)
                    P1[i] = ((P0[0] * (double)rp[i * 4] + P0[1] * (double)rp[i * 4 + 1]) + P0[2] * (double)rp[i * 4 + 2]) + c.s * (double)rp[i * 4 + 3];
                const D7 eu = ((P1[0] * fx) / P1[2] + cx) - (double)uv.x;
                const D7 ev = ((P1[1] * fy) / P1[2] + cy) - (double)uv.y;
                accumulate(A, eu, sr);
                accumulate(A, ev, sr);
                if (WB) { put_row(bo, gblk, wrow, eu); put_row(bo, gblk, wrow + 1, ev); wrow += 2; }
            }
            if (WB) put_head(bo, gblk, 3, f, kp, nres);
        }
    }
    __shared__ double red[kLinVals];
    if (lane == 0)
        for (int i = 0; i < kLinVals; ++i) red[i] = A.v[i];
    __syncwarp();
    for (int i = lane; i < kLinVals; i += 32)
        partial[((long long)blockIdx.y * partial_stride + partial_off + blockIdx.x) * kLinVals + i] = red[i];
}

__global__ void __launch_bounds__(1024)
k_lin_finish(const double *__restrict__ partial, int nchunks, double *__restrict__ out, int out_stride, const P2pView P) {
    __shared__ double tot[kLinVals];
    const int b = blockIdx.x, lane = threadIdx.x & 31, warp = threadIdx.x >> 5;
    for (int v = warp; v < kLinVals; v += 32) {
        double x = 0.0;
        for (int i = lane; i < nchunks; i += 32) x += partial[((long long)b * nchunks + i) * kLinVals + v];
        for (int o = 16; o; o >>= 1) x += __shfl_down_sync(0xffffffffu, x, o);
        if (lane == 0) tot[v] = x;
    }
    __syncthreads();
    if (threadIdx.x == 0) {
        double *o = out + (long long)b * out_stride;
        o[0] = tot[0];
        for (int a = 0; a < 7; ++a) o[1 + a] = tot[1 + a];
        int h = 8;
        for (int a = 0; a < 7; ++a)
            for (int c = a; c < 7; ++c) { o[8 + a * 7 + c] = tot[h]; o[8 + c * 7 + a] = tot[h]; ++h; }
        o[57] = tot[36]; o[58] = tot[37]; o[59] = tot[38]; o[60] = tot[39]; o[61] = tot[40];
    }
    if (P.n > 1) p2p_allreduce_record(P, b, out + (long long)b * out_stride + P.off);
}

template <class T> void dfree(T *&p) { if (p) { cudaFree(p); p = nullptr; } }

}

void lm_free(LmState &lm) {
    dfree(lm.slot_kf); dfree(lm.slot_kp); dfree(lm.flags); dfree(lm.geo2d); dfree(lm.geo3d);
    dfree(lm.idxG); dfree(lm.gpr_nb); dfree(lm.gpr_m); dfree(lm.gpr_hyper);
    dfree(lm.amap); dfree(lm.stage); dfree(lm.plane_a); dfree(lm.nnb_pos); dfree(lm.nbb); dfree(lm.nbbx); dfree(lm.nbb_m); dfree(lm.nbb_last);
    dfree(lm.idx2d); dfree(lm.idx3d); dfree(lm.d_sel); dfree(lm.d_tmp); dfree(lm.partial); dfree(lm.d_cand);
    if (lm.h_cand) cudaFreeHost(lm.h_cand);
    if (lm.h_counts) cudaFreeHost(lm.h_counts);
    if (lm.h_amap) cudaFreeHost(lm.h_amap);
    delete[] lm.n_blocks;
    if (lm.h2d_done) cudaEventDestroy(lm.h2d_done);
    if (lm.counts_done) cudaEventDestroy(lm.counts_done);
    if (lm.amap_done) cudaEventDestroy(lm.amap_done);
    lm = LmState();
}

cudaError_t lm_reserve(const DevPack &pk, const DevParams &pr, LmState &lm, int P, int lanes, cudaStream_t st) {
    cudaError_t e;
#define TRY(x) do { e = (x); if (e != cudaSuccess) { lm_free(lm); return e; } } while (0)
    const long long ns = pk.n_mp_total > 0 ? pk.n_mp_total : 1;
    if (lm.n_slots != ns || lm.P_cap < P) {
        lm_free(lm);
        const long long nsa = (ns + 15) / 16 * 16, n = nsa * P;
        lm.slot_stride = nsa;
        TRY(cudaMalloc(&lm.slot_kf, 4 * n)); TRY(cudaMalloc(&lm.slot_kp, 4 * n));
        lm.flags_bytes = (size_t)(4 * n + 16 * P);
        TRY(cudaMalloc(&lm.flags, lm.flags_bytes));
        lm.flag2d = lm.flags; lm.type3d = lm.flags + n; lm.flag3d = lm.flags + 2 * n; lm.flagG = lm.flags + 3 * n;
        lm.d_counts = reinterpret_cast<int *>(lm.flags + 4 * n);
        TRY(cudaMalloc(&lm.geo2d, 48 * n)); TRY(cudaMalloc(&lm.geo3d, 72 * n));
        TRY(cudaMalloc(&lm.idx2d, 4 * n)); TRY(cudaMalloc(&lm.idx3d, 4 * ns)); TRY(cudaMalloc(&lm.idxG, 4 * n));
        if (pr.use_gpr) { TRY(cudaMalloc(&lm.gpr_nb, 4 * n * kMaxK)); TRY(cudaMalloc(&lm.gpr_m, 4 * n)); }
        TRY(cudaMalloc(&lm.d_sel, 8));
        size_t tb = 0;
        cub::CountingInputIterator<int> it(0);
        TRY(cub::DeviceSelect::Flagged(nullptr, tb, it, lm.flag2d, lm.idx2d, lm.d_sel, (int)n, st));
        lm.tmp_bytes = tb;
        TRY(cudaMalloc(&lm.d_tmp, tb));
        TRY(cudaMallocHost(&lm.h_counts, 16 * (size_t)P));
        lm.n_blocks = new long long[4 * (size_t)P]();
        TRY(cudaEventCreateWithFlags(&lm.counts_done, cudaEventDisableTiming));
        TRY(cudaEventCreateWithFlags(&lm.amap_done, cudaEventDisableTiming));
        lm.n_slots = ns;
        lm.max_blocks = ns;
        lm.P_cap = P;
    }
    if (lanes > lm.lane_cap) {
        dfree(lm.amap); dfree(lm.stage); dfree(lm.plane_a); dfree(lm.nnb_pos); dfree(lm.nbb); dfree(lm.nbbx); dfree(lm.nbb_m); dfree(lm.nbb_last);
        if (lm.h_amap) cudaFreeHost(lm.h_amap);
        lm.h_amap = nullptr;
        lm.lane_cap = 0;
        const long long nm = ns * lanes;
        TRY(cudaMalloc(&lm.amap, sizeof(int2) * lanes)); TRY(cudaMallocHost(&lm.h_amap, sizeof(int2) * lanes));
        TRY(cudaMalloc(&lm.stage, nm)); TRY(cudaMalloc(&lm.plane_a, 32 * nm)); TRY(cudaMalloc(&lm.nnb_pos, 4 * nm));
        TRY(cudaMalloc(&lm.nbb, 4 * nm * kMaxK)); TRY(cudaMalloc(&lm.nbbx, sizeof(float4) * nm * kMaxK)); lm.nbbx_stride = nm;
        TRY(cudaMalloc(&lm.nbb_m, 4 * nm)); TRY(cudaMalloc(&lm.nbb_last, 8 * nm));
        lm.lane_cap = lanes;
        lm.h_amap[0] = make_int2(0, 0);
        TRY(cudaMemcpy(lm.amap, lm.h_amap, sizeof(int2), cudaMemcpyHostToDevice));
    }
#undef TRY
    return cudaSuccess;
}

cudaError_t lm_begin(const DevPack &pk, const DevParams &pr, LmState &lm, int P, bool partial, int lanes, cudaStream_t st) {
    cudaError_t e = lm_reserve(pk, pr, lm, P, lanes, st);
    if (e != cudaSuccess) return e;
    lm.ready = false;
    lm.clear_lanes = partial;
    if (!partial) {
        const long long n = lm.slot_stride * P;
        lm.P = P;
        lm.flag2d = lm.flags; lm.type3d = lm.flags + n; lm.flag3d = lm.flags + 2 * n; lm.flagG = lm.flags + 3 * n;
        lm.d_counts = reinterpret_cast<int *>(lm.flags + 4 * n);
        e = cudaMemsetAsync(lm.flags, 0, (size_t)(4 * n + 16 * P), st);
    }
    return e;
}

cudaError_t lm_set_lanes(LmState &lm, const int2 *lanes, int n, cudaStream_t st) {
    if (n > lm.lane_cap) return cudaErrorInvalidValue;
    lm.lane0 = lanes[0];
    if (n == 1 && lanes[0].x == lm.h_amap[0].x && lanes[0].y == lm.h_amap[0].y) return cudaSuccess;
    cudaError_t e = cudaEventSynchronize(lm.amap_done);
    if (e != cudaSuccess) return e;
    memcpy(lm.h_amap, lanes, sizeof(int2) * n);
    e = cudaMemcpyAsync(lm.amap, lm.h_amap, sizeof(int2) * n, cudaMemcpyHostToDevice, st);
    if (e == cudaSuccess) e = cudaEventRecord(lm.amap_done, st);
    return e;
}

cudaError_t lm_associate(const DevPack &pk, const DevWork &wk, const DevParams &pr, LmState &lm, int n, cudaStream_t st, bool hints, bool cert,
                         int part, bool nn_folded) {
    cudaError_t e;
#define TRY(x) do { e = (x); if (e != cudaSuccess) return e; } while (0)
    const dim3 grid((unsigned)(pk.n_sel * wk.sub), (unsigned)n);
    if (part != 2) {
        lm.ready = false;
        lm.sub = wk.sub;
        if (lm.clear_lanes) k_lm_clear<<<dim3((unsigned)((lm.slot_stride + 1023) / 1024 < 64 ? (lm.slot_stride + 1023) / 1024 : 64), (unsigned)n), 256, 0, st>>>(lm);
        if (pk.n_sel > 0) {
            if (!(pr.plane_index && !pr.use_gpr))
                k_lm_knn_a<<<grid, kWarps * 32, 0, st>>>(pk, wk, pr, lm);
            k_lm_plane_a<<<grid, 128, 0, st>>>(pk, wk, pr, lm);
        }
        TRY(cudaGetLastError());
    }
    if (part == 1 || pk.n_sel == 0) return cudaSuccess;
    if (!nn_folded) k_lm_knn_b<<<grid, kWarps * 32, 0, st>>>(pk, wk, pr, lm, hints, cert);
    k_lm_plane_b<<<grid, 128, 0, st>>>(pk, wk, pr, lm);
    TRY(cudaGetLastError());
#undef TRY
    return cudaSuccess;
}

cudaError_t lm_compact2d(LmState &lm, cudaStream_t st) {
    cub::CountingInputIterator<int> it(0);
    size_t tb = lm.tmp_bytes;
    return cub::DeviceSelect::Flagged(lm.d_tmp, tb, it, lm.flag2d, lm.idx2d, lm.d_sel, (int)(lm.slot_stride * lm.P), st);
}

cudaError_t lm_finish_associate(LmState &lm, bool use_gpr, cudaStream_t st) {
    lm.idx3d_valid = false;
    if (use_gpr) {
        cub::CountingInputIterator<int> it(0);
        size_t tb = lm.tmp_bytes;
        const cudaError_t e = cub::DeviceSelect::Flagged(lm.d_tmp, tb, it, lm.flagG, lm.idxG, lm.d_sel + 1, (int)(lm.slot_stride * lm.P), st);
        if (e != cudaSuccess) return e;
    }
    lm.counts_valid = false;
    lm.use_gpr = use_gpr;
    lm.clear_lanes = false;
    lm.ready = true;
    return cudaSuccess;
}

cudaError_t lm_compact3d(const DevPack &pk, LmState &lm, cudaStream_t st) {
    if (lm.idx3d_valid) return cudaSuccess;
    const long long ns = pk.n_mp_total > 0 ? pk.n_mp_total : 1;
    cub::CountingInputIterator<int> it(0);
    size_t tb = lm.tmp_bytes;
    const cudaError_t e = cub::DeviceSelect::Flagged(lm.d_tmp, tb, it, lm.flag3d, lm.idx3d, lm.d_counts + 1, (int)ns, st);
    if (e == cudaSuccess) lm.idx3d_valid = true;
    return e;
}

cudaError_t lm_copy_counts(LmState &lm, cudaStream_t st) {
    cudaError_t e = cudaMemcpyAsync(lm.h_counts, lm.d_counts, 16 * (size_t)lm.P, cudaMemcpyDeviceToHost, st);
    if (e == cudaSuccess) e = cudaEventRecord(lm.counts_done, st);
    return e;
}

cudaError_t lm_block_counts(LmState &lm) {
    if (!lm.ready) return cudaErrorNotReady;
    if (lm.counts_valid) return cudaSuccess;
    cudaError_t e = cudaEventSynchronize(lm.counts_done);
    if (e != cudaSuccess) return e;
    for (int p = 0; p < lm.P; ++p) {
        const int *h = lm.h_counts + 4 * p;
        long long *o = lm.n_blocks + 4 * p;
        o[0] = h[0]; o[1] = h[2]; o[2] = h[1] - h[2]; o[3] = lm.use_gpr ? h[3] : 0;
    }
    lm.counts_valid = true;
    return cudaSuccess;
}

namespace {
__global__ void k_gpr_train(const DevPack pk, const DevCand *__restrict__ c0, const LmState lm, int l0, double *__restrict__ out ,
                            int *__restrict__ out_n) {
    const int it = blockIdx.x, lane = threadIdx.x;
    const long long ms = lm.idxG[l0 + it];
    const int f = lm.slot_kf[ms];
    const int n = lm.gpr_m[ms];
    const DevKf &K = pk.kf[f];
    const DevCand &c = *c0;
    if (lane == 0) out_n[it] = n;
    double u = 0, v = 0, z = 0;
    if (lane < n) {
        const uint32_t p = lm.gpr_nb[ms * kMaxK + lane];
        double X, Y, Z;
        xform(c.R, c.t, (double)pk.px[K.pt_off + p], (double)pk.py[K.pt_off + p], (double)pk.pz[K.pt_off + p], X, Y, Z);
        u = (double)K.fx * X / Z + (double)K.cx;
        v = (double)K.fy * Y / Z + (double)K.cy;
        z = Z;
    }
    double *o = out + ((long long)it * kMaxK + lane) * 3;
    o[0] = u; o[1] = v; o[2] = z;
}
__global__ void k_gpr_scatter_hyper(const LmState lm, int l0, int nG, const double *__restrict__ fitted , double *__restrict__ hyper) {
    const int it = blockIdx.x * blockDim.x + threadIdx.x;
    if (it >= nG) return;
    const long long ms = lm.idxG[l0 + it];
    hyper[ms * 2] = fitted[it * 2];
    hyper[ms * 2 + 1] = fitted[it * 2 + 1];
}
__global__ void k_gpr_gather_hyper(const LmState lm, const DevParams pr, int nG, double *__restrict__ out ) {
    const int it = blockIdx.x * blockDim.x + threadIdx.x;
    if (it >= nG) return;
    const long long ms = lm.idxG[it];
    out[it * 2] = lm.gpr_hyper ? lm.gpr_hyper[ms * 2] : pr.gpr_sigma;
    out[it * 2 + 1] = lm.gpr_hyper ? lm.gpr_hyper[ms * 2 + 1] : pr.gpr_l;
}
}

cudaError_t lm_fit_gpr_hyper(const DevPack &pk, const DevCand *c0, const DevParams &pr, LmState &lm, int prob, cudaStream_t st, int flavour) {
    cudaError_t e = lm_block_counts(lm);
    if (e != cudaSuccess) return e;
    const int nG = (int)lm.n_blocks[4 * prob + 3];
    int l0 = 0;
    for (int q = 0; q < prob; ++q) l0 += (int)lm.n_blocks[4 * q + 3];
    if (!lm.gpr_hyper) {
        e = cudaMalloc(&lm.gpr_hyper, 16 * lm.slot_stride * lm.P_cap);
        if (e != cudaSuccess) return e;
    }
    if (nG == 0) return cudaSuccess;
    double *d_train = nullptr, *d_fit = nullptr;
    int *d_n = nullptr;
    std::vector<double> h_train((size_t)nG * kMaxK * 3), h_fit((size_t)nG * 2);
    std::vector<int> h_n(nG);
    e = cudaMalloc(&d_train, 8 * h_train.size());
    if (e == cudaSuccess) e = cudaMalloc(&d_n, 4 * (size_t)nG);
    if (e == cudaSuccess) e = cudaMalloc(&d_fit, 16 * (size_t)nG);
    if (e == cudaSuccess) {
        k_gpr_train<<<nG, kMaxK, 0, st>>>(pk, c0, lm, l0, d_train, d_n);
        e = cudaGetLastError();
    }
    if (e == cudaSuccess) e = cudaMemcpyAsync(h_train.data(), d_train, 8 * h_train.size(), cudaMemcpyDeviceToHost, st);
    if (e == cudaSuccess) e = cudaMemcpyAsync(h_n.data(), d_n, 4 * (size_t)nG, cudaMemcpyDeviceToHost, st);
    if (e == cudaSuccess) e = cudaStreamSynchronize(st);
    if (e == cudaSuccess) {
#pragma omp parallel for schedule(dynamic, 16)
        for (int it = 0; it < nG; ++it) {
            const int n = h_n[it];
            double x[kMaxK * 2], y[kMaxK];
            for (int j = 0; j < n; ++j) {
                x[j * 2] = h_train[((size_t)it * kMaxK + j) * 3];
                x[j * 2 + 1] = h_train[((size_t)it * kMaxK + j) * 3 + 1];
                y[j] = h_train[((size_t)it * kMaxK + j) * 3 + 2];
            }
            const GprFitResult r = gpr_fit(x, y, n, pr.gpr_noise, pr.gpr_sigma, pr.gpr_l, 15, flavour);
            h_fit[(size_t)it * 2] = r.sigma;
            h_fit[(size_t)it * 2 + 1] = r.l;
        }
        e = cudaMemcpyAsync(d_fit, h_fit.data(), 16 * (size_t)nG, cudaMemcpyHostToDevice, st);
    }
    if (e == cudaSuccess) {
        k_gpr_scatter_hyper<<<(nG + 127) / 128, 128, 0, st>>>(lm, l0, nG, d_fit, lm.gpr_hyper);
        e = cudaGetLastError();
    }
    if (e == cudaSuccess) e = cudaStreamSynchronize(st);
    cudaFree(d_train); cudaFree(d_n); cudaFree(d_fit);
    return e;
}

cudaError_t lm_get_gpr_hyper(const DevParams &pr, LmState &lm, double *out, cudaStream_t st) {
    cudaError_t e = lm_block_counts(lm);
    const int nG = (int)lm.n_blocks[3];
    if (e != cudaSuccess || nG == 0) return e;
    double *d = nullptr;
    e = cudaMalloc(&d, 16 * (size_t)nG);
    if (e != cudaSuccess) return e;
    k_gpr_gather_hyper<<<(nG + 127) / 128, 128, 0, st>>>(lm, pr, nG, d);
    e = cudaGetLastError();
    if (e == cudaSuccess) e = cudaMemcpyAsync(out, d, 16 * (size_t)nG, cudaMemcpyDeviceToHost, st);
    if (e == cudaSuccess) e = cudaStreamSynchronize(st);
    cudaFree(d);
    return e;
}

cudaError_t lm_stage_candidates(LmState &lm, const double *x, const int *problem, int B, cudaStream_t st) {
    cudaError_t e;
#define TRY(x) do { e = (x); if (e != cudaSuccess) return e; } while (0)
    const size_t bytes = (sizeof(LmCand) + sizeof(int)) * (size_t)B;
    if (B > lm.cand_cap) {
        dfree(lm.d_cand);
        if (lm.h_cand) cudaFreeHost(lm.h_cand);
        lm.h_cand = nullptr;
        lm.cand_cap = 0;
        TRY(cudaMalloc(&lm.d_cand, bytes));
        TRY(cudaMallocHost(&lm.h_cand, bytes));
        lm.cand_cap = B;
    }
    LmCand *hc = reinterpret_cast<LmCand *>(lm.h_cand);
    int *hp = reinterpret_cast<int *>(hc + B);
    if (!lm.h2d_done) TRY(cudaEventCreateWithFlags(&lm.h2d_done, cudaEventDisableTiming));
    TRY(cudaEventSynchronize(lm.h2d_done));
    for (int b = 0; b < B; ++b) { make_lm_candidate(x + (size_t)b * 7, hc + b); hp[b] = problem ? problem[b] : 0; }
    TRY(cudaMemcpyAsync(lm.d_cand, hc, bytes, cudaMemcpyHostToDevice, st));
    TRY(cudaEventRecord(lm.h2d_done, st));
#undef TRY
    return cudaSuccess;
}

cudaError_t lm_linearize(const DevPack &pk, const DevParams &pr, LmState &lm, const double *x, const int *problem, int B, double *d_out,
                         cudaStream_t st, const BlockOut *blocks, int out_stride, const P2pView *p2p, cudaEvent_t before_finish, bool cand_staged) {
    cudaError_t e;
#define TRY(x) do { e = (x); if (e != cudaSuccess) return e; } while (0)
    if (!cand_staged) TRY(lm_stage_candidates(lm, x, problem, B, st));
    const LmCand *cands = reinterpret_cast<const LmCand *>(lm.d_cand);
    const int *cprob = problem ? reinterpret_cast<const int *>(cands + B) : nullptr;
    const long long work = pk.sel ? (pk.n_sel_mp > 0 ? pk.n_sel_mp : 1) : lm.max_blocks;
    long long chunks_ll = (work + kLinThreads * 2 - 1) / (kLinThreads * 2);
    static const int kChunkCap = getenv("STL_LIN_CHUNKS") ? atoi(getenv("STL_LIN_CHUNKS")) : 148 * 2;
    int chunks = (int)(chunks_ll < 1 ? 1 : (chunks_ll > kChunkCap ? kChunkCap : chunks_ll));
    const long long gwork = lm.use_gpr ? work : 0;
    long long gchunks_ll = gwork > 0 ? (gwork + 3) / 4 : 0;
    int gchunks = (int)(gchunks_ll > 148 * 8 ? 148 * 8 : gchunks_ll);
    const int stride = chunks + gchunks;
    const long long need = (long long)B * stride * kLinVals;
    if (need > lm.partial_cap) {
        dfree(lm.partial);
        TRY(cudaMalloc(&lm.partial, 8 * need));
        lm.partial_cap = need;
    }
    const BlockOut bo = blocks ? *blocks : BlockOut();
    if (blocks) {
        TRY(lm_compact3d(pk, lm, st));
        k_linearize<true><<<dim3(chunks, B), kLinThreads, 0, st>>>(pk, pr, lm, cands, cprob, lm.partial, stride, bo);
    } else {
        k_linearize<false><<<dim3(chunks, B), kLinThreads, 0, st>>>(pk, pr, lm, cands, cprob, lm.partial, stride, bo);
    }
    TRY(cudaGetLastError());
    if (gchunks > 0) {
        if (blocks) k_linearize_gpr<true><<<dim3(gchunks, B), 32, 0, st>>>(pk, pr, lm, cands, cprob, lm.partial, stride, chunks, bo);
        else k_linearize_gpr<false><<<dim3(gchunks, B), 32, 0, st>>>(pk, pr, lm, cands, cprob, lm.partial, stride, chunks, bo);
        TRY(cudaGetLastError());
    }
    if (before_finish) TRY(cudaStreamWaitEvent(st, before_finish, 0));
    k_lin_finish<<<B, 1024, 0, st>>>(lm.partial, stride, d_out, out_stride > 0 ? out_stride : STL_LIN_NSUMS, p2p ? *p2p : P2pView());
    TRY(cudaGetLastError());
#undef TRY
    return cudaSuccess;
}

}
```

Before: 1076.

## Split NN and kNN neighbourhood search into separate kernels, lazy ScanView accessors

ScanView now holds a reference to the pack plus offsets and exposes accessor methods, instead of precomputing nine pointers, which should reduce register pressure in the traversal kernels. Queries are abstracted (point or shared-memory source), and stats counting moves out of the view. The neighbourhood kNN that used to run serially inside the NN kernel's per-query loop becomes its own kernel, k_nb_knn, launched with a ticket-based schedule. This spreads the kNN work across warps more evenly, at the cost of an extra launch and re-reading nn_pos from global memory.

```diff
diff --git a/spatial-temporal-lidar-camera-calibration_b200/csrc/knn.cuh b/spatial-temporal-lidar-camera-calibration_b200/csrc/knn.cuh
--- a/spatial-temporal-lidar-camera-calibration_b200/csrc/knn.cuh
+++ b/spatial-temporal-lidar-camera-calibration_b200/csrc/knn.cuh
@@ -11,26 +11,38 @@
 constexpr unsigned kFull = 0xffffffffu;
 
 struct ScanView {
-    const float *px, *py, *pz;
-    const uint32_t *orig;
-    const float4 *lo, *hi;
-    const uint16_t *adj;
-    const float *adj_cov;
-    unsigned long long *stats;
+    const DevPack &pk;
+    long long pt, node;
     int n0, n1;
-};
-
-__device__ __forceinline__ ScanView make_view(const DevPack &pk, const DevKf &K) {
-    ScanView v;
-    v.px = pk.px + K.pt_off; v.py = pk.py + K.pt_off; v.pz = pk.pz + K.pt_off;
-    v.orig = pk.orig + K.pt_off;
-    v.lo = pk.node_lo + K.node_off; v.hi = pk.node_hi + K.node_off;
-    v.adj = pk.adj ? pk.adj + K.node_off * 32 : nullptr;
-    v.adj_cov = pk.adj ? pk.adj_cov + K.node_off : nullptr;
-    v.stats = nullptr;
-    v.n0 = K.n0; v.n1 = K.n1;
-    return v;
-}
+    __device__ __forceinline__ float x(long long i) const { return pk.px[pt + i]; }
+    __device__ __forceinline__ float y(long long i) const { return pk.py[pt + i]; }
+    __device__ __forceinline__ float z(long long i) const { return pk.pz[pt + i]; }
+    __device__ __forceinline__ uint32_t orig(long long i) const { return pk.orig[pt + i]; }
+    __device__ __forceinline__ float4 lo(long long i) const { return pk.node_lo[node + i]; }
+    __device__ __forceinline__ float4 hi(long long i) const { return pk.node_hi[node + i]; }
+    __device__ __forceinline__ bool has_adj() const { return pk.adj != nullptr; }
+    __device__ __forceinline__ unsigned adj(long long leaf, int lane) const { return pk.adj[(node + leaf) * 32 + lane]; }
+    __device__ __forceinline__ float adj_cov(long long leaf) const { return pk.adj_cov[node + leaf]; }
+};
+
+__device__ __forceinline__ ScanView make_view(const DevPack &pk, const DevKf &K) { return ScanView{pk, K.pt_off, K.node_off, K.n0, K.n1}; }
+
+__device__ __forceinline__ void bump(unsigned long long *stats, int i, int lane) {
+    if (stats && lane == 0) atomicAdd(stats + i, 1ull);
+}
+
+struct QPoint {
+    double x_, y_, z_;
+    __device__ __forceinline__ double x() const { return x_; }
+    __device__ __forceinline__ double y() const { return y_; }
+    __device__ __forceinline__ double z() const { return z_; }
+};
+struct QShared {
+    const volatile double *p;
+    __device__ __forceinline__ double x() const { return p[0]; }
+    __device__ __forceinline__ double y() const { return p[1]; }
+    __device__ __forceinline__ double z() const { return p[2]; }
+};
 
 struct QueryF { float xl, xh, yl, yh, zl, zh; };
 __device__ __forceinline__ QueryF make_queryf(double x, double y, double z) {
@@ -61,24 +73,25 @@
     }
     __device__ __forceinline__ void note_bound(float b) { g2 = fminf(g2, b); }
     __device__ __forceinline__ void seed(const ScanView &S, uint32_t p, double qx, double qy, double qz) {
-        const double dd = dist3e(qx, qy, qz, (double)S.px[p], (double)S.py[p], (double)S.pz[p]);
-        if (dd == dd) { d = dd; df = __double2float_ru(dd); oi = S.orig[p]; pos = p; }
-    }
-    __device__ __forceinline__ void visit(const ScanView &S, int leaf, double qx, double qy, double qz, int lane) {
+        const double dd = dist3e(qx, qy, qz, (double)S.x(p), (double)S.y(p), (double)S.z(p));
+        if (dd == dd) { d = dd; df = __double2float_ru(dd); oi = S.orig(p); pos = p; }
+    }
+    template <class Q>
+    __device__ __forceinline__ void visit(const ScanView &S, int leaf, const Q &q, int lane) {
         const int g = leaf * kLeaf + lane;
-        const double dd = dist3e(qx, qy, qz, (double)S.px[g], (double)S.py[g], (double)S.pz[g]);
+        const double dd = dist3e(q.x(), q.y(), q.z(), (double)S.x(g), (double)S.y(g), (double)S.z(g));
         const float lowf = dd == dd ? below(dd) : __int_as_float(0x7f800000);
-        const bool q = dd <= d;
-        if (!__any_sync(kFull, q)) {
+        const bool le = dd <= d;
+        if (!__any_sync(kFull, le)) {
             note_pruned(lowf, (uint32_t)g != pos);
             return;
         }
-        const uint32_t o = q ? S.orig[g] : 0xffffffffu;
-        unsigned hi = q ? (unsigned)__double2hiint(dd) : 0xffffffffu;
+        const uint32_t o = le ? S.orig(g) : 0xffffffffu;
+        unsigned hi = le ? (unsigned)__double2hiint(dd) : 0xffffffffu;
         const unsigned mhi = __reduce_min_sync(kFull, hi);
-        unsigned lo = (q && hi == mhi) ? (unsigned)__double2loint(dd) : 0xffffffffu;
+        unsigned lo = (le && hi == mhi) ? (unsigned)__double2loint(dd) : 0xffffffffu;
         const unsigned mlo = __reduce_min_sync(kFull, lo);
-        const bool tie = q && hi == mhi && (unsigned)__double2loint(dd) == mlo;
+        const bool tie = le && hi == mhi && (unsigned)__double2loint(dd) == mlo;
         const unsigned mo = __reduce_min_sync(kFull, tie ? o : 0xffffffffu);
         const double cd = __hiloint2double((int)mhi, (int)mlo);
         if (cd < d || (cd == d && mo < oi)) {
@@ -110,13 +123,14 @@
     __device__ __forceinline__ bool may_contain(float lb) const { return lb <= r2f && (count < k || lb <= wdf); }
     __device__ __forceinline__ void note_pruned(float, bool) {}
     __device__ __forceinline__ void note_bound(float) {}
-    __device__ __forceinline__ void visit(const ScanView &S, int leaf, double qx, double qy, double qz, int lane) {
+    template <class Q>
+    __device__ __forceinline__ void visit(const ScanView &S, int leaf, const Q &q, int lane) {
         const int g = leaf * kLeaf + lane;
-        const double dd = dist3e(qx, qy, qz, (double)S.px[g], (double)S.py[g], (double)S.pz[g]);
+        const double dd = dist3e(q.x(), q.y(), q.z(), (double)S.x(g), (double)S.y(g), (double)S.z(g));
         const bool pre = dd < r2 && (count < k || dd <= wd);
         unsigned mask = __ballot_sync(kFull, pre);
         if (!mask) return;
-        const uint32_t o = pre ? S.orig[g] : 0xffffffffu;
+        const uint32_t o = pre ? S.orig(g) : 0xffffffffu;
         if (__popc(mask) >= (count == 0 ? 4 : 8)) {
             bulk_merge(pre ? dd : (double)INFINITY, o, (uint32_t)g, lane);
             return;
@@ -197,13 +211,10 @@
     }
 };
 
-template <class Sink>
-__device__ __forceinline__ void traverse(const ScanView &S, double qx, double qy, double qz, Sink &sink, int lane, int first_leaf = -1) {
-    if (first_leaf >= 0) sink.visit(S, first_leaf, qx, qy, qz, lane);
-    const float4 *lo2 = S.lo + S.n0 + S.n1, *hi2 = S.hi + S.n0 + S.n1;
-    const float4 *lo1 = S.lo + S.n0, *hi1 = S.hi + S.n0;
-    const QueryF qf = make_queryf(qx, qy, qz);
-    const float lb2 = box_lbf(qf, lo2[lane], hi2[lane]);
+template <class Sink, class Q>
+__device__ __forceinline__ void traverse(const ScanView &S, const Q &q, Sink &sink, int lane, int first_leaf = -1) {
+    if (first_leaf >= 0) sink.visit(S, first_leaf, q, lane);
+    const float lb2 = box_lbf(make_queryf(q.x(), q.y(), q.z()), S.lo(S.n0 + S.n1 + lane), S.hi(S.n0 + S.n1 + lane));
     const unsigned key2 = __float_as_uint(lb2);
     unsigned done2 = 0;
     for (;;) {
@@ -213,7 +224,7 @@
         const int s2 = __ffs(__ballot_sync(kFull, c2 && key2 == m2)) - 1;
         done2 |= 1u << s2;
         const int n1i = s2 * 32 + lane;
-        const float lb1 = box_lbf(qf, lo1[n1i], hi1[n1i]);
+        const float lb1 = box_lbf(make_queryf(q.x(), q.y(), q.z()), S.lo(S.n0 + n1i), S.hi(S.n0 + n1i));
         const unsigned key1 = __float_as_uint(lb1);
         unsigned done1 = 0;
         for (;;) {
@@ -223,7 +234,7 @@
             const int s1 = __ffs(__ballot_sync(kFull, c1 && key1 == m1)) - 1;
             done1 |= 1u << s1;
             const int n0i = (s2 * 32 + s1) * 32 + lane;
-            const float lb0 = box_lbf(qf, S.lo[n0i], S.hi[n0i]);
+            const float lb0 = box_lbf(make_queryf(q.x(), q.y(), q.z()), S.lo(n0i), S.hi(n0i));
             const unsigned key0 = __float_as_uint(lb0);
             unsigned done0 = ((s2 * 32 + s1) == (first_leaf >> 5) && first_leaf >= 0) ? (1u << (first_leaf & 31)) : 0u;
             for (;;) {
@@ -232,13 +243,18 @@
                 if (m0 == 0xffffffffu) break;
                 const int s0 = __ffs(__ballot_sync(kFull, c0 && key0 == m0)) - 1;
                 done0 |= 1u << s0;
-                sink.visit(S, (s2 * 32 + s1) * 32 + s0, qx, qy, qz, lane);
+                sink.visit(S, (s2 * 32 + s1) * 32 + s0, q, lane);
             }
             sink.note_pruned(lb0, !((done0 >> lane) & 1u));
         }
         sink.note_pruned(lb1, !((done1 >> lane) & 1u));
     }
     sink.note_pruned(lb2, !((done2 >> lane) & 1u));
+}
+
+template <class Sink>
+__device__ __forceinline__ void traverse(const ScanView &S, double qx, double qy, double qz, Sink &sink, int lane, int first_leaf = -1) {
+    traverse(S, QPoint{qx, qy, qz}, sink, lane, first_leaf);
 }
 
 __device__ __forceinline__ int next_ticket(int *ticket, int lane) {
@@ -247,14 +263,14 @@
     return __shfl_sync(kFull, t, 0);
 }
 
-template <class Sink>
-__device__ __forceinline__ float scan_adjacent(const ScanView &S, int home, double qx, double qy, double qz, Sink &sink, int lane) {
-    if (S.adj == nullptr) return -1.f;
-    const float cov = S.adj_cov[home];
+template <class Sink, class Q>
+__device__ __forceinline__ float scan_adjacent(const ScanView &S, int home, const Q &q, Sink &sink, int lane) {
+    if (!S.has_adj()) return -1.f;
+    const float cov = S.adj_cov(home);
     if (cov < 0.f) return -1.f;
-    const unsigned id = S.adj[(long long)home * 32 + lane];
-    const QueryF qf = make_queryf(qx, qy, qz);
-    const float lb = id != 0xffffu ? box_lbf(qf, S.lo[id], S.hi[id]) : __int_as_float(0x7f800000);
+    const unsigned id = S.adj(home, lane);
+    const QueryF qf = make_queryf(q.x(), q.y(), q.z());
+    const float lb = id != 0xffffu ? box_lbf(qf, S.lo(id), S.hi(id)) : __int_as_float(0x7f800000);
     const unsigned key = __float_as_uint(lb);
     unsigned done = 0;
     for (;;) {
@@ -263,24 +279,25 @@
         if (m == 0xffffffffu) break;
         const int s = __ffs(__ballot_sync(kFull, c && key == m)) - 1;
         done |= 1u << s;
-        sink.visit(S, (int)__shfl_sync(kFull, id, s), qx, qy, qz, lane);
+        sink.visit(S, (int)__shfl_sync(kFull, id, s), q, lane);
     }
     sink.note_pruned(lb, !((done >> lane) & 1u));
     return cov;
 }
 
-__device__ __forceinline__ void knn_around_point(const ScanView &S, uint32_t pos, SinkK &kn, int lane) {
-    const double x = (double)S.px[pos], y = (double)S.py[pos], z = (double)S.pz[pos];
-    const float cov = scan_adjacent(S, (int)(pos >> 5), x, y, z, kn, lane);
+__device__ __forceinline__ void knn_around_point(const ScanView &S, uint32_t pos, SinkK &kn, int lane, unsigned long long *stats = nullptr) {
+    const double x = (double)S.x(pos), y = (double)S.y(pos), z = (double)S.z(pos);
+    const float cov = scan_adjacent(S, (int)(pos >> 5), QPoint{x, y, z}, kn, lane);
     const bool done = cov > 3.0e38f || (cov >= 0.f && kn.count == kn.k && kn.wdf < cov);
-    if (S.stats && lane == 0) { atomicAdd(S.stats + 0, 1ull); atomicAdd(S.stats + (done ? 1 : (cov >= 0.f ? 2 : 3)), 1ull); }
+    bump(stats, 0, lane);
+    bump(stats, done ? 1 : (cov >= 0.f ? 2 : 3), lane);
     if (done) return;
     if (cov >= 0.f) kn = SinkK(kn.k, kn.r2);
     traverse(S, x, y, z, kn, lane, (int)(pos >> 5));
 }
 
 __device__ __forceinline__ float home_box_delta(const ScanView &S, int home, double qx, double qy, double qz) {
-    const float4 lo = S.lo[home], hi = S.hi[home];
+    const float4 lo = S.lo(home), hi = S.hi(home);
     const float xl = __double2float_rd(qx), xh = __double2float_ru(qx), yl = __double2float_rd(qy), yh = __double2float_ru(qy);
     const float zl = __double2float_rd(qz), zh = __double2float_ru(qz);
     const float gx = fmaxf(fmaxf(__fsub_ru(lo.x, xl), __fsub_ru(xh, hi.x)), 0.f);
@@ -289,40 +306,41 @@
     return __fsqrt_ru(__fadd_ru(__fadd_ru(__fmul_ru(gx, gx), __fmul_ru(gy, gy)), __fmul_ru(gz, gz)));
 }
 
-__device__ __forceinline__ void nn_near_leaf_seeded(const ScanView &S, float adj_r, int home, double qx, double qy, double qz, Sink1 &nn,
-                                                    int lane, float delta) {
-    const float cov = scan_adjacent(S, home, qx, qy, qz, nn, lane);
-    if (S.stats && lane == 0) atomicAdd(S.stats + 4, 1ull);
+template <class Q>
+__device__ __forceinline__ bool nn_adjacent(const ScanView &S, float adj_r, int home, const Q &q, Sink1 &nn, int lane,
+                                            float delta, unsigned long long *stats) {
+    const float cov = scan_adjacent(S, home, q, nn, lane);
+    bump(stats, 4, lane);
     if (cov >= 0.f && nn.pos != 0xffffffffu) {
         const float reach = __fadd_ru(__fsqrt_ru(nn.df), delta);
         if (cov > 3.0e38f ? reach <= adj_r : reach < __fsqrt_rd(cov)) {
-            if (S.stats && lane == 0) atomicAdd(S.stats + 5, 1ull);
+            bump(stats, 5, lane);
             const float u = __fsub_rd(cov > 3.0e38f ? adj_r : __fsqrt_rd(cov), delta);
             nn.note_bound(u > 0.f ? __fmul_rd(u, u) : 0.f);
-            return;
+            return true;
         }
         const int l1 = (int)(nn.pos >> 5);
         if (l1 != home) {
-            const float cov1 = S.adj_cov[l1];
+            const float cov1 = S.adj_cov(l1);
             const float two_rho = __fmul_ru(2.f, __fsqrt_ru(nn.df));
             if (cov1 >= 0.f && (cov1 > 3.0e38f ? two_rho <= adj_r : two_rho < __fsqrt_rd(cov1))) {
                 const float rho_up = __fsqrt_ru(nn.df);
-                scan_adjacent(S, l1, qx, qy, qz, nn, lane);
-                if (S.stats && lane == 0) atomicAdd(S.stats + 5, 1ull);
+                scan_adjacent(S, l1, q, nn, lane);
+                bump(stats, 5, lane);
                 const float u = __fsub_rd(cov1 > 3.0e38f ? adj_r : __fsqrt_rd(cov1), rho_up);
                 nn.note_bound(u > 0.f ? __fmul_rd(u, u) : 0.f);
-                return;
+                return true;
             }
         }
     }
-    if (S.stats && lane == 0) atomicAdd(S.stats + (cov >= 0.f ? 6 : 7), 1ull);
-    traverse(S, qx, qy, qz, nn, lane);
+    bump(stats, cov >= 0.f ? 6 : 7, lane);
+    return false;
 }
 
 __device__ __forceinline__ void nn_near_leaf(const ScanView &S, float adj_r, int home, double qx, double qy, double qz, Sink1 &nn,
-                                             int lane, uint32_t hint = 0xffffffffu) {
+                                             int lane, uint32_t hint = 0xffffffffu, unsigned long long *stats = nullptr) {
     if (hint != 0xffffffffu) nn.seed(S, hint, qx, qy, qz);
-    nn_near_leaf_seeded(S, adj_r, home, qx, qy, qz, nn, lane, home_box_delta(S, home, qx, qy, qz));
+    if (!nn_adjacent(S, adj_r, home, QPoint{qx, qy, qz}, nn, lane, home_box_delta(S, home, qx, qy, qz), stats)) traverse(S, qx, qy, qz, nn, lane);
 }
 
 struct PlaneOut { V3 n; double reg; int m; bool gates_ok; };
@@ -332,7 +350,7 @@
     const uint32_t *__restrict__ nb;
     __device__ __forceinline__ void get(int j, double &x, double &y, double &z) const {
         const uint32_t p = nb[j];
-        x = (double)S.px[p]; y = (double)S.py[p]; z = (double)S.pz[p];
+        x = (double)S.x(p); y = (double)S.y(p); z = (double)S.z(p);
     }
 };
 struct NbCoords {
@@ -346,7 +364,7 @@
 __device__ __forceinline__ void store_nb_coords(float4 *__restrict__ nbx, long long stride, long long slot, const ScanView &S, int lane,
                                                 int count, uint32_t kpos) {
     float4 v = make_float4(0.f, 0.f, 0.f, 0.f);
-    if (lane < count) v = make_float4(S.px[kpos], S.py[kpos], S.pz[kpos], __uint_as_float(kpos));
+    if (lane < count) v = make_float4(S.x(kpos), S.y(kpos), S.z(kpos), __uint_as_float(kpos));
     nbx[(long long)lane * stride + slot] = v;
 }
 
diff --git a/spatial-temporal-lidar-camera-calibration_b200/csrc/knn3d.cu b/spatial-temporal-lidar-camera-calibration_b200/csrc/knn3d.cu
--- a/spatial-temporal-lidar-camera-calibration_b200/csrc/knn3d.cu
+++ b/spatial-temporal-lidar-camera-calibration_b200/csrc/knn3d.cu
@@ -27,9 +27,162 @@
     xform(c.Ri, c.ti, cxm, cym, czm, qx, qy, qz);
 }
 
+__device__ __forceinline__ void twin_point(const DevPack &pk, const DevKf &K, const DevCand &c, int f, uint32_t kp, double &lx, double &ly,
+                                           double &lz) {
+    const float *Tcw = pk.Tcw + (long long)f * 12;
+    const float *mp = pk.kp_mp + (K.kp_off + kp) * 3;
+    const double ma = (double)mp[0], mb = (double)mp[1], mc = (double)mp[2];
+    const double Mx = dadd(dot3e((double)Tcw[0], (double)Tcw[1], (double)Tcw[2], ma, mb, mc), (double)Tcw[3]);
+    const double My = dadd(dot3e((double)Tcw[4], (double)Tcw[5], (double)Tcw[6], ma, mb, mc), (double)Tcw[7]);
+    const double Mz = dadd(dot3e((double)Tcw[8], (double)Tcw[9], (double)Tcw[10], ma, mb, mc), (double)Tcw[11]);
+    xform(c.Ri, c.ti, dmul(Mx, c.s), dmul(My, c.s), dmul(Mz, c.s), lx, ly, lz);
+}
+__device__ __forceinline__ bool twin_settled(const ScanView &S, double qx, double qy, double qz, double lx, double ly, double lz, uint32_t out_pos,
+                                             float out_g2, double &nn_d) {
+    if (out_pos == 0xffffffffu) return false;
+    const double move = sqrt(dist3e(qx, qy, qz, lx, ly, lz)) * (1.0 + 1e-9) + 1e-12;
+    const double dh = dist3e(lx, ly, lz, (double)S.x(out_pos), (double)S.y(out_pos), (double)S.z(out_pos));
+    const double reach = (double)__fsqrt_rd(out_g2) - move;
+    nn_d = dh;
+    return reach > 0.0 && reach * reach > dh * (1.0 + 1e-6) + 1e-18;
+}
+__device__ __forceinline__ void twin_store(const DevParams &pr, uint32_t *lm_pos, int *lm_m, long long slot, double nn_d, uint32_t nn_p, uint32_t hint) {
+    if (nn_d > pr.max_3d_dist2) {
+        lm_pos[slot] = 0xffffffffu;
+    } else {
+        lm_pos[slot] = nn_p;
+        lm_m[slot] = nn_p == hint ? -2 : -3;
+    }
+}
+
+constexpr int kMaxBatch = 8;
+struct QueryRec {
+    double x, y, z;
+    double d;
+    uint32_t oi, pos;
+    float g2;
+    uint32_t hint;
+    float delta;
+    uint32_t out_pos;
+    float out_g2;
+    int pad;
+};
+__device__ __forceinline__ void load_sink(const QueryRec &r, Sink1 &nn) {
+    nn.d = r.d; nn.oi = r.oi; nn.pos = r.pos; nn.g2 = r.g2;
+    if (nn.pos != 0xffffffffu) nn.df = __double2float_ru(nn.d);
+}
+
 __global__ void __launch_bounds__(kWarps * 32, STL_KNN_MINB)
-k_nn_knn(const DevPack pk, const DevWork wk, const DevParams pr, const int B, const int batch, uint32_t *__restrict__ lm_pos,
+k_nn_knn(__grid_constant__ const DevPack pk, const DevWork wk, const DevParams pr, const int B, const int batch, uint32_t *__restrict__ lm_pos,
          int *__restrict__ lm_m) {
+    struct Unit { long long cbase, qbase; int f, b, bf, j, nq; };
+    __shared__ Unit unit;
+    __shared__ int ticket;
+    __shared__ QueryRec recs[kWarps][kMaxBatch];
+    struct WarpState { int t0; unsigned todo; };
+    __shared__ WarpState wstate[kWarps];
+    if (threadIdx.x == 0) {
+        const int sub = wk.sub, j = blockIdx.x % sub, bf = blockIdx.x / sub;
+        const int fi = bf / B, f = sel_kf(pk, fi), b = bf - fi * B;
+        unit = Unit{(long long)b * pk.n_kp_total + pk.kf[f].kp_off, (long long)b * pk.n_mp_total + pk.kf[f].mp_off, f, b, bf, j,
+                    wk.n_q[(long long)b * pk.n_kf + f]};
+        ticket = 0;
+    }
+    __syncthreads();
+    const volatile Unit &u = unit;
+    if (u.nq <= 0) return;
+    const int lane = threadIdx.x & 31;
+    const ScanView S = make_view(pk, pk.kf[u.f]);
+    QueryRec *R = recs[threadIdx.x >> 5];
+    volatile WarpState &w = wstate[threadIdx.x >> 5];
+    for (;;) {
+        {
+            const int t0 = next_ticket(&ticket, lane) * batch;
+            if ((long long)t0 * wk.sub + u.j >= u.nq) break;
+            w.t0 = t0;
+        }
+        if (lane < batch && (w.t0 + lane) * wk.sub + u.j < u.nq) {
+            const int qi = (w.t0 + lane) * wk.sub + u.j;
+            QueryRec &r = R[lane];
+            const uint2 ks = wk.q_kpsp[u.cbase + qi];
+            const uint32_t hint = ks.y;
+            double qx, qy, qz;
+            map_point_lidar(pk, pk.kf[u.f], wk.cand[u.b], u.f, ks.x, qx, qy, qz);
+            r.x = qx; r.y = qy; r.z = qz;
+            r.hint = hint;
+            const double dd = dist3e(qx, qy, qz, (double)S.x(hint), (double)S.y(hint), (double)S.z(hint));
+            const bool ok = dd == dd;
+            r.d = ok ? dd : DBL_MAX; r.oi = ok ? S.orig(hint) : 0xffffffffu; r.pos = ok ? hint : 0xffffffffu;
+            r.g2 = HUGE_VALF;
+            r.delta = home_box_delta(S, (int)(hint >> 5), qx, qy, qz);
+        }
+        {
+            const unsigned vmask = __ballot_sync(kFull, lane < batch && (w.t0 + lane) * wk.sub + u.j < u.nq);
+            w.todo = vmask;
+        }
+        __syncwarp();
+        while (w.todo) {
+            const int src = __ffs(w.todo) - 1;
+            QueryRec &r = R[src];
+            Sink1 nn;
+            load_sink(r, nn);
+            if (!nn_adjacent(S, pr.adj_r, (int)(r.hint >> 5), QShared{&r.x}, nn, lane, r.delta, wk.dbg_stats)) traverse(S, QShared{&r.x}, nn, lane);
+            __syncwarp();
+            if (lane == 0) {
+                r.out_pos = nn.pos;
+                r.out_g2 = nn.g2;
+                w.todo = w.todo & (w.todo - 1);
+            }
+            __syncwarp();
+        }
+        auto query = [&]() { return (w.t0 + lane) * wk.sub + u.j; };
+        auto valid = [&]() { return lane < batch && query() < u.nq; };
+        if (valid()) {
+            const int qi = query();
+            wk.nn_pos[u.qbase + qi] = R[lane].out_pos;
+            wk.nn_g2[u.qbase + qi] = R[lane].out_g2;
+        }
+        if (lm_pos != nullptr && u.b == 0) {
+            bool need = false;
+            if (valid()) {
+                const int qi = query();
+                QueryRec &r = R[lane];
+                double lx, ly, lz, nn_d;
+                twin_point(pk, pk.kf[u.f], wk.cand[0], u.f, wk.q_kpsp[u.cbase + qi].x, lx, ly, lz);
+                need = !twin_settled(S, r.x, r.y, r.z, lx, ly, lz, r.out_pos, r.out_g2, nn_d);
+                if (!need) { r.pos = r.out_pos; r.d = nn_d; }
+                r.x = lx; r.y = ly; r.z = lz;
+            }
+            {
+                const unsigned nmask = __ballot_sync(kFull, need);
+                w.todo = nmask;
+            }
+            __syncwarp();
+            while (w.todo) {
+                const int src = __ffs(w.todo) - 1;
+                QueryRec &r = R[src];
+                const uint32_t h = r.out_pos != 0xffffffffu ? r.out_pos : r.hint;
+                Sink1 nn;
+                nn.seed(S, h, r.x, r.y, r.z);
+                const int home = (int)(h >> 5);
+                if (!nn_adjacent(S, pr.adj_r, home, QShared{&r.x}, nn, lane, home_box_delta(S, home, r.x, r.y, r.z), wk.dbg_stats))
+                    traverse(S, QShared{&r.x}, nn, lane);
+                __syncwarp();
+                if (lane == 0) {
+                    r.pos = nn.pos;
+                    r.d = nn.d;
+                    w.todo = w.todo & (w.todo - 1);
+                }
+                __syncwarp();
+            }
+            if (valid()) twin_store(pr, lm_pos, lm_m, pk.kf[u.f].mp_off + query(), R[lane].d, R[lane].pos, R[lane].hint);
+        }
+        __syncwarp();
+    }
+}
+
+__global__ void __launch_bounds__(kWarps * 32, STL_KNN_MINB)
+k_nb_knn(const DevPack pk, const DevWork wk, const DevParams pr, const int B) {
     const int sub = wk.sub;
     const int j = blockIdx.x % sub;
     const int bf = blockIdx.x / sub;
@@ -38,97 +191,21 @@
     if (nq <= 0) return;
     const int lane = threadIdx.x & 31;
     const DevKf K = pk.kf[f];
-    const DevCand &c = wk.cand[b];
-    ScanView S = make_view(pk, K);
-    S.stats = wk.dbg_stats;
-    const long long cbase = (long long)b * pk.n_kp_total + K.kp_off;
+    const ScanView S = make_view(pk, K);
     const long long qbase = (long long)b * pk.n_mp_total + K.mp_off;
     __shared__ int ticket;
     if (threadIdx.x == 0) ticket = 0;
     __syncthreads();
     for (;;) {
-        const int t0 = next_ticket(&ticket, lane) * batch;
-        if ((long long)t0 * sub + j >= nq) break;
-        const int qi = (t0 + lane) * sub + j;
-        const bool valid = lane < batch && qi < nq;
-        double qx = 0, qy = 0, qz = 0, sd = DBL_MAX;
-        uint32_t hint = 0, soi = 0xffffffffu, spos = 0xffffffffu;
-        float delta = 0.f;
-        if (valid) {
-            const uint2 ks = wk.q_kpsp[cbase + qi];
-            hint = ks.y;
-            map_point_lidar(pk, K, c, f, ks.x, qx, qy, qz);
-            const double dd = dist3e(qx, qy, qz, (double)S.px[hint], (double)S.py[hint], (double)S.pz[hint]);
-            if (dd == dd) { sd = dd; soi = S.orig[hint]; spos = hint; }
-            delta = home_box_delta(S, (int)(hint >> 5), qx, qy, qz);
-        }
-        uint32_t out_pos = 0xffffffffu;
-        float out_g2 = 0.f;
-        unsigned todo = __ballot_sync(kFull, valid);
-        while (todo) {
-            const int src = __ffs(todo) - 1;
-            todo &= todo - 1;
-            const double x = __shfl_sync(kFull, qx, src), y = __shfl_sync(kFull, qy, src), z = __shfl_sync(kFull, qz, src);
-            const uint32_t h = __shfl_sync(kFull, hint, src);
-            Sink1 nn;
-            nn.d = __shfl_sync(kFull, sd, src);
-            nn.oi = __shfl_sync(kFull, soi, src);
-            nn.pos = __shfl_sync(kFull, spos, src);
-            if (nn.pos != 0xffffffffu) nn.df = __double2float_ru(nn.d);
-            nn_near_leaf_seeded(S, pr.adj_r, (int)(h >> 5), x, y, z, nn, lane, __shfl_sync(kFull, delta, src));
-            if (lane == src) { out_pos = nn.pos; out_g2 = nn.g2; }
-            if (pr.use_plane && !pr.plane_index) {
-                const long long slot = qbase + (long long)(t0 + src) * sub + j;
-                SinkK kn(pr.k, pr.radius2);
-                knn_around_point(S, nn.pos, kn, lane);
-                wk.nb[slot * kMaxK + lane] = lane < kn.count ? kn.kpos : 0xffffffffu;
-                store_nb_coords(wk.nbx, wk.nbx_stride, slot, S, lane, kn.count, kn.kpos);
-                const double last = __shfl_sync(kFull, kn.kd, kn.count > 0 ? kn.count - 1 : 0);
-                if (lane == 0) { wk.nb_m[slot] = kn.count; wk.nb_last[slot] = last; }
-            }
-        }
-        if (valid) { wk.nn_pos[qbase + qi] = out_pos; wk.nn_g2[qbase + qi] = out_g2; }
-        if (lm_pos != nullptr && b == 0) {
-            double lx = 0, ly = 0, lz = 0, nn_d = DBL_MAX;
-            uint32_t nn_p = 0xffffffffu;
-            bool need = false;
-            if (valid) {
-                const float *Tcw = pk.Tcw + (long long)f * 12;
-                const float *mp = pk.kp_mp + (K.kp_off + wk.q_kpsp[cbase + qi].x) * 3;
-                const double ma = (double)mp[0], mb = (double)mp[1], mc = (double)mp[2];
-                const double Mx = dadd(dot3e((double)Tcw[0], (double)Tcw[1], (double)Tcw[2], ma, mb, mc), (double)Tcw[3]);
-                const double My = dadd(dot3e((double)Tcw[4], (double)Tcw[5], (double)Tcw[6], ma, mb, mc), (double)Tcw[7]);
-                const double Mz = dadd(dot3e((double)Tcw[8], (double)Tcw[9], (double)Tcw[10], ma, mb, mc), (double)Tcw[11]);
-                xform(c.Ri, c.ti, dmul(Mx, c.s), dmul(My, c.s), dmul(Mz, c.s), lx, ly, lz);
-                need = true;
-                if (out_pos != 0xffffffffu) {
-                    const double move = sqrt(dist3e(qx, qy, qz, lx, ly, lz)) * (1.0 + 1e-9) + 1e-12;
-                    const double dh = dist3e(lx, ly, lz, (double)S.px[out_pos], (double)S.py[out_pos], (double)S.pz[out_pos]);
-                    const double reach = (double)__fsqrt_rd(out_g2) - move;
-                    if (reach > 0.0 && reach * reach > dh * (1.0 + 1e-6) + 1e-18) { need = false; nn_p = out_pos; nn_d = dh; }
-                }
-            }
-            unsigned todo2 = __ballot_sync(kFull, need);
-            while (todo2) {
-                const int src = __ffs(todo2) - 1;
-                todo2 &= todo2 - 1;
-                const double x = __shfl_sync(kFull, lx, src), y = __shfl_sync(kFull, ly, src), z = __shfl_sync(kFull, lz, src);
-                uint32_t h = __shfl_sync(kFull, out_pos, src);
-                if (h == 0xffffffffu) h = __shfl_sync(kFull, hint, src);
-                Sink1 nn;
-                nn_near_leaf(S, pr.adj_r, (int)(h >> 5), x, y, z, nn, lane, h);
-                if (lane == src) { nn_p = nn.pos; nn_d = nn.d; }
-            }
-            if (valid) {
-                const long long slot = K.mp_off + qi;
-                if (nn_d > pr.max_3d_dist2) {
-                    lm_pos[slot] = 0xffffffffu;
-                } else {
-                    lm_pos[slot] = nn_p;
-                    lm_m[slot] = nn_p == hint ? -2 : -3;
-                }
-            }
-        }
+        const int qi = next_ticket(&ticket, lane) * sub + j;
+        if (qi >= nq) break;
+        const long long slot = qbase + qi;
+        SinkK kn(pr.k, pr.radius2);
+        knn_around_point(S, wk.nn_pos[slot], kn, lane, wk.dbg_stats);
+        wk.nb[slot * kMaxK + lane] = lane < kn.count ? kn.kpos : 0xffffffffu;
+        store_nb_coords(wk.nbx, wk.nbx_stride, slot, S, lane, kn.count, kn.kpos);
+        const double last = __shfl_sync(kFull, kn.kd, kn.count > 0 ? kn.count - 1 : 0);
+        if (lane == 0) { wk.nb_m[slot] = kn.count; wk.nb_last[slot] = last; }
     }
 }
 
@@ -152,7 +229,7 @@
             double qx, qy, qz;
             map_point_lidar(pk, K, c, f, kp, qx, qy, qz);
             const uint32_t np = wk.nn_pos[qbase + qi];
-            const double nx = (double)S.px[np], ny = (double)S.py[np], nz = (double)S.pz[np];
+            const double nx = (double)S.x(np), ny = (double)S.y(np), nz = (double)S.z(np);
             const double dx = dsub(nx, qx), dy = dsub(ny, qy), dz = dsub(nz, qz);
             double dist = sqrt(dot3e(dx, dy, dz, dx, dy, dz));
             int is_plane = 0, m = 0;
@@ -172,13 +249,13 @@
             c3d += 1.0;
             if (debug) {
                 const long long o = K.kp_off + qi;
-                wk.dbg_nn[o] = S.orig[np];
+                wk.dbg_nn[o] = S.orig(np);
                 wk.dbg_m[o] = m;
                 wk.dbg_plane[o] = is_plane;
                 wk.dbg_dist[o] = dist;
                 for (int t = 0; t < kMaxK; ++t) {
                     const uint32_t p = (pr.use_plane && !pr.plane_index && t < m) ? wk.nb[(qbase + qi) * kMaxK + t] : 0xffffffffu;
-                    wk.dbg_knn[o * kMaxK + t] = p == 0xffffffffu ? 0xffffffffu : S.orig[p];
+                    wk.dbg_knn[o * kMaxK + t] = p == 0xffffffffu ? 0xffffffffu : S.orig(p);
                 }
             }
         }
@@ -242,7 +319,7 @@
         int mm = -1;
         if (p < K.n_pts) {
             const long long o = K.pt_off - first_pt + p;
-            const PlaneOut po = plane_thread(S, nb + o * kMaxK, nb_m[o], nb_last[o], (double)S.px[p], (double)S.py[p], (double)S.pz[p], pr, pr.variant == 1);
+            const PlaneOut po = plane_thread(S, nb + o * kMaxK, nb_m[o], nb_last[o], (double)S.x(p), (double)S.y(p), (double)S.z(p), pr, pr.variant == 1);
             r.nx = po.n.x; r.ny = po.n.y; r.nz = po.n.z; r.reg = po.reg;
             mm = po.gates_ok ? po.m : -(po.m + 1);
         }
@@ -291,8 +368,10 @@
     if (B <= 0) return cudaSuccess;
     if (pk.n_sel <= 0) return after_traversal ? cudaEventRecord(after_traversal, st) : cudaSuccess;
     int batch = (long long)pk.n_sel * B >= 600 ? 8 : 4;
-    if (const char *e = getenv("STL_K2_BATCH")) batch = std::max(1, std::min(32, atoi(e)));
-    k_nn_knn<<<(unsigned)(pk.n_sel * B * wk.sub), kWarps * 32, 0, st>>>(pk, wk, pr, B, batch, lm_pos, lm_m);
+    if (const char *e = getenv("STL_K2_BATCH")) batch = std::max(1, std::min(kMaxBatch, atoi(e)));
+    const unsigned units = (unsigned)(pk.n_sel * B * wk.sub);
+    k_nn_knn<<<units, kWarps * 32, 0, st>>>(pk, wk, pr, B, batch, lm_pos, lm_m);
+    if (pr.use_plane && !pr.plane_index) k_nb_knn<<<units, kWarps * 32, 0, st>>>(pk, wk, pr, B);
     cudaError_t e = cudaGetLastError();
     if (e != cudaSuccess) return e;
     if (after_traversal && (e = cudaEventRecord(after_traversal, st)) != cudaSuccess) return e;
diff --git a/spatial-temporal-lidar-camera-calibration_b200/csrc/lm.cu b/spatial-temporal-lidar-camera-calibration_b200/csrc/lm.cu
--- a/spatial-temporal-lidar-camera-calibration_b200/csrc/lm.cu
+++ b/spatial-temporal-lidar-camera-calibration_b200/csrc/lm.cu
@@ -121,7 +121,7 @@
             m = wk.nb_m[slot];
             if (m < 0) continue;
         }
-        const double cx = (double)S.px[sp], cy = (double)S.py[sp], cz = (double)S.pz[sp];
+        const double cx = (double)S.x(sp), cy = (double)S.y(sp), cz = (double)S.z(sp);
         const PlaneOut po = from_index ? plane_lookup(pk, K, sp)
                                        : plane_fit(NbCoords{wk.nbx + slot, wk.nbx_stride}, m, wk.nb_last[slot], cx, cy, cz, pr);
         if (!po.gates_ok) continue;
@@ -190,7 +190,7 @@
                 double ox, oy, oz;
                 xform(c0.Ri, c0.ti, ex, ey, ez, ox, oy, oz);
                 const double move = sqrt(dist3e(ox, oy, oz, qx, qy, qz)) * (1.0 + 1e-9) + 1e-12;
-                const double dh = dist3e(qx, qy, qz, (double)S.px[hint], (double)S.py[hint], (double)S.pz[hint]);
+                const double dh = dist3e(qx, qy, qz, (double)S.x(hint), (double)S.y(hint), (double)S.z(hint));
                 const double reach = (double)__fsqrt_rd(nn_g2[slot]) - move;
                 if (reach > 0.0 && reach * reach > dh * (1.0 + 1e-6) + 1e-18) { settled = true; nn_pos = hint; nn_d = dh; }
             }
```

Measured after the change: 1098, median of 6. 1.02x the previous value.
